# jedison-github/gentun

Hardware: AMD Instinct MI355X
Metric: candidates/hour + best val-acc@genN, Genetic-CNN CIFAR-10 1/2/4/8 GPU (higher is better)
Workload: dtype fp32

## Files before the change

### csrc/hip/cnn_args.h

```cpp
#pragma once
#include "common.h"

template <typename F>
static void lds_limit(F* fn, size_t bytes) {
  if (bytes > 65536) (void)hipFuncSetAttribute(reinterpret_cast<const void*>(fn), hipFuncAttributeMaxDynamicSharedMemorySize,
                                         (int)bytes);
}

struct GroupRec {
  int g;
  int in_mask;
  int out_mask;
  int pad;
};

#define GT_MAXSLOT 8

struct ConvArgs {
  const void* in[GT_MAXSLOT];
  const void* mask;
  const int64_t* gather;
  const StepState* st;
  void* out[GT_MAXSLOT];
  const void* out_mask[GT_MAXSLOT];
  const uint16_t* w;
  const float* bias;
  const GroupRec* gtab;
  int n_in, n_out, acc_flags, relu;
  int G, B, H, W, Cinp, Coutp, KH, KW, TH;
  int ngroups;
  void* xsum;
  int dbg;
  int epi_bf16;
  int prec;
  long wps;
  int cbb;
  void* pool_y;
  uint8_t* pool_mask;
  void* unpool_x1;
  const int* unpool_sel;
  int cout_real;
  int Hr, Wr;
  int wino;
  int wfrag;
};

__device__ __forceinline__ GroupRec group_rec(const GroupRec* gtab, int y, int n_in, int n_out, int acc,
                                              const void* const* out_mask) {
  if (gtab) return gtab[y];
  GroupRec r;
  r.g = y;
  r.in_mask = (1 << n_in) - 1;
  int rm = 0;
  for (int k = 0; k < n_out; ++k)
    if (out_mask && out_mask[k]) rm |= 1 << k;
  r.out_mask = ((1 << n_out) - 1) | ((acc & 0xff) << 8) | (rm << 16);
  r.pad = 0;
  return r;
}

struct WgradArgs {
  const void* in[GT_MAXSLOT];
  const int64_t* gather;
  const StepState* st;
  const void* dz;
  float* part_w;
  float* part_b;
  const GroupRec* gtab;
  int n_in;
  int G, B, H, W, Cinp, Coutp, KH, KW, S, pps;
  int ngroups;
  int prec;
  int cout_real;
};

__device__ __forceinline__ bool pos_bits(uint32_t h) { return h != 0u && h < 0x8000u; }
```

### csrc/hip/cnn_conv_fast.hip

```cpp
#include "conv_fast_host.h"

FastSwitches g_fast;

static int swap_switch(int& sw, int v) {
  const int old = sw;
  sw = v;
  return old;
}

extern "C" int gt_conv_set_s2in_ct1(int on) { return swap_switch(g_fast.s2in_ct1, on); }

extern "C" int gt_conv_set_regepi(int on) { return swap_switch(g_fast.regepi, on); }

extern "C" int gt_conv_set_smallq(int on) { return swap_switch(g_fast.smallq, on); }

static int smallq_th(const ConvArgs* a, int TH, int THMIN) {
  if (!g_fast.smallq) return TH;
  int th = TH;
  while (th > THMIN && (long)a->ngroups * a->B * (a->H / th) < g_fast.smallq_wg) th >>= 1;
  return th;
}

static bool pk_ok(const ConvArgs* a, int nt) {
  const int last = a->cout_real - 16 * (nt - 1);
  return a->prec == 1 && a->cout_real > 0 && last >= 1 && last <= 4;
}

static const std::vector<ConvRow>& conv_rows() {
  static const std::vector<ConvRow> rows = {
    {8, 4, {tile<5, 5, 1, 32, 4, 2, 3, 2, 1, 1>(IF_TH | IF_PK), tile<5, 5, 1, 32, 4, 2, 3, 2, 1>(IF_TH),
            tile<5, 5, 1, 32, 8, 2, 3, 4, 1, 1>(IF_PK), tile<5, 5, 1, 32, 8, 2, 3, 4, 1>()}},
    {8, 4, {tile<3, 3, 3, 32, 4, 2, 3, 2, 1, 1>(IF_TH | IF_PK), tile<3, 3, 3, 32, 4, 2, 3, 2, 1>(IF_TH),
            tile<3, 3, 3, 32, 8, 2, 3, 4, 1, 1>(IF_PK), tile<3, 3, 3, 32, 8, 2, 3, 4, 1>()}},
    {8, 2, {tile<5, 5, 3, 16, 4, 4, 7, 4, 1>(IF_TH), ct1<5, 5, 3, 16, 2, 4, 7, 4>(IF_TH), ct1<5, 5, 3, 16, 8, 4, 7, 4, 0>()}},
    {8, 2, {tile<3, 3, 7, 16, 4, 4, 7, 4, 1>(IF_TH), ct1<3, 3, 7, 16, 2, 4, 7, 4>(IF_TH), ct1<3, 3, 7, 16, 8, 4, 7, 4, 0>()}},
    {8, 4, {ct1<5, 5, 7, 16, 4, 2, 3, 4>(IF_S2CT1 | IF_TH), ct1<5, 5, 7, 16, 8, 2, 3, 4>(IF_S2CT1),
            tile<5, 5, 7, 16, 8, 2, 3, 4, 1, 1>(IF_PK), tile<5, 5, 7, 16, 8, 2, 3, 4, 1>()}},
    {8, 8, {tile<5, 5, 7, 8, 8, 7, 13, 7, 1>()}},
    {8, 8, {tile<3, 3, 13, 8, 8, 7, 13, 7, 1>()}},
    {8, 8, {tile<5, 5, 13, 8, 8, 4, 7, 4, 1>()}},
    {8, 8, {tile<5, 5, 1, 32, 8, 4, 8, 4, 1>()}},
    {4, 4, {ct1<3, 3, 8, 32, 4, 4, 8, 4, 0>()}},
    {8, 8, {ct1<5, 5, 8, 16, 8, 8, 16, 8, 0>()}},
    {8, 8, {ct1<3, 3, 16, 16, 8, 8, 16, 8, 0>()}},
    {4, 4, {tile<5, 5, 16, 16, 4, 4, 8, 4, 1>()}},
    {8, 8, {tile<5, 5, 16, 8, 8, 16, 32, 8, 1>()}},
    {8, 8, {tile<3, 3, 32, 8, 8, 16, 32, 8, 1>()}},
    {4, 4, {tile<5, 5, 32, 8, 4, 8, 16, 4, 1>()}},
    {8, 8, {tile<5, 5, 1, 32, 8, 2, 3, 4, 0>()}},
    {8, 8, {tile<3, 3, 3, 32, 8, 2, 3, 4, 0>()}},
    {16, 16, {tile<5, 5, 3, 16, 16, 4, 7, 4, 0>()}},
    {16, 16, {tile<3, 3, 7, 16, 16, 4, 7, 8, 0>()}},
    {16, 16, {tile<5, 5, 7, 16, 16, 2, 3, 4, 0>()}},
    {8, 8, {tile<5, 5, 7, 8, 8, 7, 13, 7, 0>()}},
    {8, 8, {tile<3, 3, 13, 8, 8, 7, 13, 7, 0>()}},
    {8, 8, {tile<5, 5, 13, 8, 8, 4, 7, 4, 0>()}},
  };
  return rows;
}

struct ConvChoice {
  const ConvKernel* k;
  dim3 grid;
  unsigned block;
  size_t lds;
};

static bool variant_ok(const ConvArgs* a, const ConvRow& r, const ConvVariant& v) {
  return (!(v.cond & IF_TH) || smallq_th(a, r.hmod, r.thmin) == v.k.TH) && (!(v.cond & IF_PK) || pk_ok(a, v.k.NT)) &&
         (!(v.cond & IF_RE) || g_fast.regepi) && (!(v.cond & IF_S2CT1) || g_fast.s2in_ct1);
}

static bool select_conv(const ConvArgs* a, ConvChoice* c) {
  if (a->mask) return false;
  for (const std::vector<ConvRow>* rows : {&conv_rows(), &conv_rows_ext()})
    for (const ConvRow& r : *rows) {
      const ConvKernel& g = r.v[0].k;
      if (a->KH != g.KH || a->KW != g.KW || a->Cinp != g.NCBI * 8 || a->W != g.W || a->Coutp != g.NCO * 8 ||
          a->prec != g.PREC || a->H % r.hmod != 0)
        continue;
      for (const ConvVariant& v : r.v)
        if (variant_ok(a, r, v)) {
          *c = {&v.k, dim3(a->B * (a->H / v.k.TH), a->ngroups), (unsigned)v.k.NWV * 64,
                (size_t)(a->epi_bf16 != 0 ? v.k.lds_fwd : v.k.lds_bwd)};
          return true;
        }
    }
  return false;
}

static int launch_fast(const void* fn, dim3 grid, unsigned block, size_t lds, const void* args, hipStream_t stream) {
  lds_limit(fn, lds);
  void* kargs[] = {const_cast<void*>(args)};
  (void)hipLaunchKernel(fn, grid, dim3(block), kargs, lds, stream);
  return (int)hipGetLastError();
}

extern "C" int gt_conv_wino(const ConvArgs* a, hipStream_t stream, int probe);

extern "C" int gt_conv_fast(const ConvArgs* a, hipStream_t stream) {
  if (a->wino) return gt_conv_wino(a, stream, 0);
  if (a->mask) return -100;
  if (a->prec != 0 && a->prec != 1) return -1;
  ConvChoice c;
  if (!select_conv(a, &c)) return -100;
  return launch_fast(c.k->fn, c.grid, c.block, c.lds, a, stream);
}

static int probe_rows(const ConvArgs* a) {
  if (a->wino) {
    const int rc = gt_conv_wino(a, nullptr, 1);
    return rc >= 1000 ? rc - 1000 : 0;
  }
  ConvChoice c;
  return select_conv(a, &c) ? c.k->TH : 0;
}

extern "C" int gt_conv_fast_probe(const ConvArgs* a) {
  const int th = probe_rows(a);
  return th % 2 == 0 ? th : 0;
}

extern "C" int gt_conv_fast_probe_any(const ConvArgs* a) { return probe_rows(a) > 0 ? 1 : 0; }

struct ConvSel {
  int KH, KW, NCBI, W, TH, NT, NCO, NWV, PREC, PK, RE, CTX, SCH, lds_fwd, lds_bwd;
  int gx, gy, gz, block, lds;
};
extern "C" int gt_conv_fast_select(const ConvArgs* a, ConvSel* s) {
  ConvChoice c;
  if (a->wino || (a->prec != 0 && a->prec != 1) || !select_conv(a, &c)) return 0;
  const ConvKernel& k = *c.k;
  *s = {k.KH, k.KW, k.NCBI, k.W, k.TH, k.NT, k.NCO, k.NWV, k.PREC, k.PK, k.RE, k.CTX, k.SCH, k.lds_fwd, k.lds_bwd,
        (int)c.grid.x, (int)c.grid.y, (int)c.grid.z, (int)c.block, (int)c.lds};
  return 1;
}
extern "C" size_t gt_sizeof_conv_sel() { return sizeof(ConvSel); }

__global__ void __launch_bounds__(256) wgrad_reduce_kernel(WgradArgs a) {
  const GroupRec gr = group_rec(a.gtab, blockIdx.y, a.n_in, 0, 0, nullptr);
  const int g = gr.g;
  const long kd = (long)a.KH * a.KW * a.Cinp;
  const long n = (long)a.Coutp * kd;
  const long gs = (long)a.G * n;
  float* pw = a.part_w + (long)g * n;
  const long i4 = ((long)blockIdx.x * 256 + threadIdx.x) * 4;
  if (i4 < n) {
    float4 acc = make_float4(0.f, 0.f, 0.f, 0.f);
    int sp = 0;
    for (; sp + 8 <= a.S; sp += 8) {
      float4 v[8];
#pragma unroll
      for (int k = 0; k < 8; ++k) v[k] = *reinterpret_cast<const float4*>(pw + (long)(sp + k) * gs + i4);
#pragma unroll
      for (int k = 0; k < 8; ++k) { acc.x += v[k].x; acc.y += v[k].y; acc.z += v[k].z; acc.w += v[k].w; }
    }
    for (; sp < a.S; ++sp) {
      const float4 v = *reinterpret_cast<const float4*>(pw + (long)sp * gs + i4);
      acc.x += v.x; acc.y += v.y; acc.z += v.z; acc.w += v.w;
    }
    *reinterpret_cast<float4*>(pw + i4) = acc;
  }
  if (blockIdx.x == 0 && a.part_b) {
    float* pb = a.part_b + (long)g * a.Coutp;
    for (int i = threadIdx.x; i < a.Coutp; i += 256) {
      float acc = 0.f;
      for (int sp = 0; sp < a.S; ++sp) acc += pb[(long)sp * a.G * a.Coutp + i];
      pb[i] = acc;
    }
  }
}

extern "C" int gt_wgrad_reduce(const WgradArgs* a, hipStream_t stream) {
  const long n = (long)a->Coutp * a->KH * a->KW * a->Cinp;
  if (n % 4 || a->S < 2) return -1;
  dim3 grid((unsigned)((n / 4 + 255) / 256), a->ngroups);
  hipLaunchKernelGGL(wgrad_reduce_kernel, grid, dim3(256), 0, stream, *a);
  return (int)hipGetLastError();
}

extern "C" int gt_wgrad_set_nb(int nb) { return swap_switch(g_fast.wgrad_nb, nb); }

extern "C" int gt_wgrad_set_nz(int nz) { return swap_switch(g_fast.wgrad_nz, nz); }

static int wgrad_nz(const WgradArgs* a) {
  const int force = g_fast.wgrad_nz;
  if (force == 1 || force == 2 || force == 4 || force == 8) return force;
  const int blocks = a->S * a->ngroups;
  return blocks < 64 ? 4 : blocks < 160 ? 2 : 1;
}

static bool wgrad_pk_ok(const WgradArgs* a, int mt) {
  const int last = a->cout_real - 16 * (mt - 1);
  return a->cout_real > 0 && last >= 1 && last <= 4;
}

static const std::vector<WgradRow>& wgrad_rows() {
  static const std::vector<WgradRow> rows = {
    wgrad_f32<5, 5, 1, 3, 32, 8, 4, 1>(),
    wgrad_f32<3, 3, 3, 3, 32, 4, 4, 1>(),
    wgrad_f32<5, 5, 3, 7, 16, 4, 8, 1>(),
    wgrad_f32<3, 3, 7, 7, 16, 4, 8, 1>(),
    wgrad_f32z<5, 5, 7, 13, 8, 4, 8, 4>(),
    wgrad_f32z<3, 3, 13, 13, 8, 4, 8, 4>(),
    wgrad_f32<5, 5, 1, 8, 32, 4, 4, 1>(),
    wgrad_f32<3, 3, 8, 8, 32, 2, 8, 1>(),
    wgrad_f32z<5, 5, 8, 16, 16, 2, 8, 7>(),
    wgrad_f32z<3, 3, 16, 16, 16, 2, 8, 4>(),
    wgrad_f32z<5, 5, 16, 32, 8, 4, 8, 13>(),
    wgrad_f32z<3, 3, 32, 32, 8, 4, 8, 10>(),
    wgrad_bf16<5, 5, 1, 3, 32, 8, 4, 1>(),
    wgrad_bf16<3, 3, 3, 3, 32, 8, 4, 1>(),
    wgrad_bf16<5, 5, 3, 7, 16, 16, 8, 2>(),
    wgrad_bf16<3, 3, 7, 7, 16, 16, 8, 2>(),
  };
  return rows;
}

static const WgradRow* wgrad_row(int KH, int KW, int Cinp, int Coutp, int H, int W, int prec) {
  for (const std::vector<WgradRow>* rows : {&wgrad_rows(), &wgrad_rows_ext()})
    for (const WgradRow& r : *rows)
      if (KH == r.KH && KW == r.KW && Cinp == r.NCBI * 8 && Coutp == r.NCBO * 8 && W == r.W && prec == r.PREC &&
          H % r.R == 0)
        return &r;
  return nullptr;
}

struct WgradChoice {
  const WgradKernel* k;
  dim3 grid;
  unsigned block;
};

static bool select_wgrad(const WgradArgs* a, WgradChoice* c) {
  const WgradRow* r = wgrad_row(a->KH, a->KW, a->Cinp, a->Coutp, a->H, a->W, a->prec);
  if (!r || a->pps % (r->R * r->W) != 0) return false;
  const int nz = r->NZ ? r->NZ : wgrad_nz(a);
  const int pk = r->PREC == 1 && wgrad_pk_ok(a, (r->NCBO * 8 + 15) / 16) ? 1 : 0;
  int nw = r->NW, nb = 1;
  if (r->NZ == 0 && nz == 2) nb = r->NB;
  else if (r->NZ == 0 && nz == 8) nw = 4;
  else if (nz == 1) nb = (g_fast.wgrad_nb ? g_fast.wgrad_nb : r->NB) == 1 ? 1 : 2;
  for (const WgradKernel& k : r->k)
    if (k.NW == nw && k.NB == nb && k.PK == pk && k.NZ == nz) {
      *c = {&k, dim3(a->S, a->ngroups, nz), (unsigned)nw * 64};
      return true;
    }
  return false;
}

extern "C" int gt_wgrad_fast_band(int KH, int KW, int Cinp, int Coutp, int H, int W, int prec) {
  const WgradRow* r = wgrad_row(KH, KW, Cinp, Coutp, H, W, prec);
  return r ? r->R * r->W : 0;
}

extern "C" int gt_wgrad_fast_splits(int KH, int KW, int Cinp, int Coutp, int H, int W, int prec) {
  (void)KH; (void)KW; (void)Cinp; (void)Coutp; (void)H;
  if (prec == 1) {
    return W >= 32 ? 32 : W <= 8 ? 4 : 8;
  }
  return W >= 32 ? 16 : 3;
}

extern "C" int gt_wgrad_fast(const WgradArgs* a, hipStream_t stream) {
  if (a->prec != 0 && a->prec != 1) return -1;
  WgradChoice c;
  if (!select_wgrad(a, &c)) return -100;
  return launch_fast(c.k->fn, c.grid, c.block, 0, a, stream);
}

struct WgradSel {
  int KH, KW, NCBI, NCBO, W, R, NW, NB, PK, NZ, PREC;
  int gx, gy, gz, block, lds;
};
extern "C" int gt_wgrad_fast_select(const WgradArgs* a, WgradSel* s) {
  WgradChoice c;
  if (!select_wgrad(a, &c)) return 0;
  const WgradKernel& k = *c.k;
  *s = {k.KH, k.KW, k.NCBI, k.NCBO, k.W, k.R, k.NW, k.NB, k.PK, k.NZ, k.PREC,
        (int)c.grid.x, (int)c.grid.y, (int)c.grid.z, (int)c.block, 0};
  return 1;
}
extern "C" size_t gt_sizeof_wgrad_sel() { return sizeof(WgradSel); }

extern "C" int gt_conv_frag_order(int KH, int KW, int NCBI, int W, int prec, int* out, int n) {
  const int NCH = KH * KW * NCBI;
  const bool parts = prec == 1 && NCBI == 7 && W == 16 && KH == 3 && KW == 3;
  for (int e = 0; e < n; ++e) {
    int kk, cb;
    if (e >= NCH) { out[e] = -1; continue; }
    if (parts) {
      const int E0 = KH * KW * 4;
      if (e < E0) { kk = e >> 2; cb = e & 3; }
      else { const int e1 = e - E0; kk = e1 / 3; cb = 4 + e1 - kk * 3; }
    } else {
      kk = e / NCBI; cb = e - kk * NCBI;
    }
    out[e] = kk * NCBI + cb;
  }
  return (NCH + 3) / 4;
}

struct FragSeg {
  const float* w;
  uint16_t* dst;
  const int* order;
  long ps;
  int Q, Cop, Cip, KH, KW;
  int NT, NKS, NCBIc;
  int dgrad;
  int npl;
};

struct FragArgs {
  const FragSeg* segs;
  const int2* blocks;
};

__global__ void __launch_bounds__(256) conv_wfrag_kernel(FragArgs a) {
  const int2 blk = a.blocks[blockIdx.x];
  const FragSeg s = a.segs[blk.x];
  const long item = (long)blk.y + threadIdx.x;
  if (item >= (long)s.Q * s.NT * s.NKS * 64) return;
  const int lane = (int)(item & 63);
  long r = item >> 6;
  const int ks = (int)(r % s.NKS); r /= s.NKS;
  const int t = (int)(r % s.NT);
  const int q = (int)(r / s.NT);
  const int row = t * 16 + (lane & 15), e = ks * 4 + (lane >> 4);
  const int nat = s.order[e];
  float v[8];
#pragma unroll
  for (int j = 0; j < 8; ++j) v[j] = 0.f;
  if (nat >= 0) {
    const int kk = nat / s.NCBIc, cb = nat - kk * s.NCBIc;
    const int kh = kk / s.KW, kw = kk - kh * s.KW;
    if (!s.dgrad && row < s.Cop) {
      const float* src = s.w + ((((long)q * s.Cop + row) * s.KH + kh) * s.KW + kw) * s.Cip + cb * 8;
#pragma unroll
      for (int j = 0; j < 8; ++j) v[j] = src[j];
    } else if (s.dgrad && row < s.Cip) {
      const int khl = s.KH - 1 - kh, kwl = s.KW - 1 - kw;
#pragma unroll
      for (int j = 0; j < 8; ++j)
        v[j] = s.w[((((long)q * s.Cop + cb * 8 + j) * s.KH + khl) * s.KW + kwl) * s.Cip + row];
    }
  }
  uint16_t* d = s.dst + item * 8;
  if (s.npl == 1) {
    *reinterpret_cast<uint4*>(d) = pack8(v);
    return;
  }
  uint4 p0, p1, p2;
  split8(v, p0, p1, p2);
  *reinterpret_cast<uint4*>(d) = p0;
  *reinterpret_cast<uint4*>(d + s.ps) = p1;
  *reinterpret_cast<uint4*>(d + 2 * s.ps) = p2;
}

extern "C" int gt_conv_wfrag(const void* av, int nblocks, hipStream_t stream) {
  if (nblocks < 1) return 0;
  hipLaunchKernelGGL(conv_wfrag_kernel, dim3(nblocks), dim3(256), 0, stream, *static_cast<const FragArgs*>(av));
  return (int)hipGetLastError();
}

extern "C" size_t gt_sizeof_frag_seg() { return sizeof(FragSeg); }
```

### csrc/hip/conv_fast_host.h

```cpp
#pragma once
#include <initializer_list>
#include <vector>

#include "conv_fast_impl.h"

struct FastSwitches {
  int s2in_ct1 = 1;
  int regepi = 1;
  int smallq = 1;
  long smallq_wg = 300;
  int wgrad_nb = 0;
  int wgrad_nz = 0;
};
extern FastSwitches g_fast;

struct ConvKernel {
  int KH, KW, NCBI, W, TH, NT, NCO, NWV, PREC, PK, RE, CTX, SCH;
  int lds_fwd, lds_bwd;
  const void* fn;
};

template <int KH, int KW, int NCBI, int W, int TH, int NT, int NCO, int NWV, int PREC, int PK = 0, int RE = 0,
          int CTX = 0, int SCH = 0>
static ConvKernel conv_kernel() {
  static_assert((NCO * 8 + 15) / 16 == NT, "NT co tiles of 16 cover the NCO chunks of 8 channels");
  using Cfg = FastCfg<KH, KW, NCBI, W, TH, NT, NCO, PREC>;
  return {KH, KW, NCBI, W, TH, NT, NCO, NWV, PREC, PK, RE, CTX, SCH, (int)Cfg::lds(true), (int)Cfg::lds(false),
          reinterpret_cast<const void*>(&conv_fast_kernel<KH, KW, NCBI, W, TH, NT, NCO, NWV, PREC, PK, RE, CTX, SCH>)};
}

enum : int {
  IF_TH = 1,
  IF_PK = 2,
  IF_RE = 4,
  IF_S2CT1 = 8,
};

struct ConvVariant {
  int cond;
  ConvKernel k;
};
typedef std::vector<ConvVariant> ConvVariants;

template <int KH, int KW, int NCBI, int W, int TH, int NT, int NCO, int NWV, int PREC, int PK = 0>
static ConvVariants tile(int cond = 0) {
  ConvVariants v;
  if (PREC == 1 && W % 16 == 0) v.push_back({cond | IF_RE, conv_kernel<KH, KW, NCBI, W, TH, NT, NCO, NWV, PREC, PK, 1>()});
  v.push_back({cond, conv_kernel<KH, KW, NCBI, W, TH, NT, NCO, NWV, PREC, PK, 0>()});
  return v;
}

template <int KH, int KW, int NCBI, int W, int TH, int NT, int NCO, int NWV, int SCH = 1>
static ConvVariants ct1(int cond = 0) {
  return {{cond, conv_kernel<KH, KW, NCBI, W, TH, NT, NCO, NWV, 1, 0, 1, 1, SCH>()}};
}

struct ConvRow {
  int hmod, thmin;
  ConvVariants v;
  ConvRow(int hmod_, int thmin_, std::initializer_list<ConvVariants> parts) : hmod(hmod_), thmin(thmin_) {
    for (const ConvVariants& p : parts) v.insert(v.end(), p.begin(), p.end());
  }
};

struct WgradKernel {
  int KH, KW, NCBI, NCBO, W, R, NW, NB, PK, NZ, PREC;
  const void* fn;
};

template <int KH, int KW, int NCBI, int NCBO, int W, int R, int NW, int NB, int PK = 0, int NZ = 1>
static WgradKernel wgrad_kernel_f32() {
  return {KH, KW, NCBI, NCBO, W, R, NW, NB, PK, NZ, 1,
          reinterpret_cast<const void*>(&wgrad_fast_f32_kernel<KH, KW, NCBI, NCBO, W, R, NW, NB, PK, NZ>)};
}
template <int KH, int KW, int NCBI, int NCBO, int W, int R, int NW, int NB>
static WgradKernel wgrad_kernel_bf16() {
  return {KH, KW, NCBI, NCBO, W, R, NW, NB, 0, 1, 0,
          reinterpret_cast<const void*>(&wgrad_fast_kernel<KH, KW, NCBI, NCBO, W, R, NW, NB>)};
}

struct WgradRow {
  int KH, KW, NCBI, NCBO, W, R, NW, PREC;
  int NB;
  int NZ;
  std::vector<WgradKernel> k;
};

template <int KH, int KW, int NCBI, int NCBO, int W, int R, int NW, int NB>
static WgradRow wgrad_f32() {
  return {KH, KW, NCBI, NCBO, W, R, NW, 1, NB, 0,
          {wgrad_kernel_f32<KH, KW, NCBI, NCBO, W, R, NW, 1, 0>(), wgrad_kernel_f32<KH, KW, NCBI, NCBO, W, R, NW, 1, 1>(),
           wgrad_kernel_f32<KH, KW, NCBI, NCBO, W, R, NW, 2, 0>(), wgrad_kernel_f32<KH, KW, NCBI, NCBO, W, R, NW, 2, 1>(),
           wgrad_kernel_f32<KH, KW, NCBI, NCBO, W, R, NW, NB, 0, 2>(), wgrad_kernel_f32<KH, KW, NCBI, NCBO, W, R, NW, NB, 1, 2>(),
           wgrad_kernel_f32<KH, KW, NCBI, NCBO, W, R, NW, 1, 0, 4>(), wgrad_kernel_f32<KH, KW, NCBI, NCBO, W, R, NW, 1, 1, 4>(),
           wgrad_kernel_f32<KH, KW, NCBI, NCBO, W, R, 4, 1, 0, 8>(), wgrad_kernel_f32<KH, KW, NCBI, NCBO, W, R, 4, 1, 1, 8>()}};
}
template <int KH, int KW, int NCBI, int NCBO, int W, int R, int NW, int NZ>
static WgradRow wgrad_f32z() {
  return {KH, KW, NCBI, NCBO, W, R, NW, 1, 1, NZ,
          {wgrad_kernel_f32<KH, KW, NCBI, NCBO, W, R, NW, 1, 0, NZ>(), wgrad_kernel_f32<KH, KW, NCBI, NCBO, W, R, NW, 1, 1, NZ>()}};
}
template <int KH, int KW, int NCBI, int NCBO, int W, int R, int NW, int NB>
static WgradRow wgrad_bf16() {
  return {KH, KW, NCBI, NCBO, W, R, NW, 0, NB, 1,
          {wgrad_kernel_bf16<KH, KW, NCBI, NCBO, W, R, NW, 1>(), wgrad_kernel_bf16<KH, KW, NCBI, NCBO, W, R, NW, 2>()}};
}

const std::vector<ConvRow>& conv_rows_ext();
const std::vector<WgradRow>& wgrad_rows_ext();
```

### csrc/hip/conv_fast_impl.h

```cpp
#pragma once

#include <algorithm>
#include <cstdio>
#include <cstdlib>
#include <type_traits>

#include "cnn_args.h"


__device__ __forceinline__ int opaque_i(int x) {
  asm volatile("" : "+v"(x));
  return x;
}

template <int KH, int KW, int NCBI, int W, int PREC>
struct S2Parts {
  static constexpr bool on = PREC == 1 && NCBI == 7 && W == 16 && KH == 3 && KW == 3;
  static constexpr int e0 = KH * KW * 4;
};

template <int KH, int KW, int NCBI, int W, int TH, int NT, int NCO, int PREC>
struct FastCfg {
  static constexpr int NPL = PREC ? GT_NPL_F32 : 1;
  static constexpr int PW = W + KW - 1;
  static constexpr int NP = (TH + KH - 1) * PW * NCBI;
  static constexpr int NCBP = NCBI + ((NCBI & 1) ? 0 : 1);
  static constexpr int NPIX = (TH + KH - 1) * PW;
  static constexpr int PPR = (S2Parts<KH, KW, NCBI, W, PREC>::on || NCBI == 3) ? 5 : (NCBI % 2 == 0) ? (NCBI == 4 ? 4 : 2) : 6;
  static constexpr int PP2 = 2 * NPIX + ((PPR - (2 * NPIX) % 8) + 8) % 8;
  static constexpr int TP = TH * W;
  static constexpr int OROW = NT * 16 + 4;
  static constexpr int OROWB = NT * 16 + 8;
  static constexpr int NPL_ = PREC ? GT_NPL_F32 : 1;
  static constexpr long OTILE = (long)TP * OROW * 4;
  static constexpr long LDS_PM = (long)NPIX * NCBP * 16 * NPL_ > OTILE ? (long)NPIX * NCBP * 16 * NPL_ : OTILE;
  static constexpr long LDS_PR = (long)((NCBI + 1) / 2) * PP2 * 16 * NPL_ > OTILE ? (long)((NCBI + 1) / 2) * PP2 * 16 * NPL_ : OTILE;
  static constexpr long LDS_CU = 160 * 1024;
  static constexpr bool PAIR = PREC == 1 && NCBI >= 2 && LDS_CU / LDS_PR >= LDS_CU / LDS_PM;
  static constexpr int PXS = PAIR ? 2 : NCBP;
  static constexpr int NPP = PAIR ? ((NCBI + 1) / 2) * PP2 : NPIX * NCBP;
  __host__ __device__ static constexpr int cbo(int cb) { return PAIR ? (cb >> 1) * PP2 + (cb & 1) : cb; }
  static size_t lds(bool fwd) {
    const size_t p = (size_t)NPP * 16 * NPL;
    const size_t o = (fwd && !PREC) ? (size_t)TP * OROWB * 2 : (size_t)TP * OROW * 4;
    return p > o ? p : o;
  }
};

template <int TH, int W, int NCO, int NTH, int PREC, typename LD>
__device__ __forceinline__ void fused_pool(const ConvArgs& a, LD ld, int g, int b, int h0, int tid) {
  typedef typename ActT<PREC>::T AT;
  constexpr int WO = W / 2, NPP = (TH / 2) * WO * NCO;
  static_assert(TH % 2 == 0 && W % 2 == 0, "pooled tiles need even rows / columns");
  const int Ho = a.H >> 1;
  const long n = (long)g * a.B + b;
  for (int i = tid; i < NPP; i += NTH) {
    const int cb = i % NCO, pp = i / NCO, pr = pp / WO, pc = pp - pr * WO;
    const int p0 = 2 * pr * W + 2 * pc;
    float m[8], t[8];
    int arg[8] = {0, 0, 0, 0, 0, 0, 0, 0};
    ld(p0, cb, m);
    const int offs[3] = {1, W, W + 1};
#pragma unroll
    for (int q = 0; q < 3; ++q) {
      ld(p0 + offs[q], cb, t);
#pragma unroll
      for (int j = 0; j < 8; ++j)
        if (t[j] > m[j]) { m[j] = t[j]; arg[j] = q + 1; }
    }
    const long o = ((n * Ho + (h0 >> 1) + pr) * WO + pc) * (NCO * 8) + cb * 8;
    st_chunk(static_cast<AT*>(a.pool_y) + o, m);
    if (a.pool_mask) {
      uint32_t lo = 0, hi = 0;
#pragma unroll
      for (int j = 0; j < 4; ++j) lo |= (uint32_t)(arg[j] | (m[j] > 0.f ? 4 : 0)) << (8 * j);
#pragma unroll
      for (int j = 0; j < 4; ++j) hi |= (uint32_t)(arg[4 + j] | (m[4 + j] > 0.f ? 4 : 0)) << (8 * j);
      *reinterpret_cast<uint2*>(a.pool_mask + o) = make_uint2(lo, hi);
    }
  }
}

template <typename AT>
__device__ __forceinline__ void unpool_chunk(const ConvArgs& a, int g, long n, int h, int w, int cb, const float* v) {
  const int Cp = a.Coutp, H2 = 2 * a.H, W2 = 2 * a.W;
  const long o = ((n * a.H + h) * a.W + w) * Cp + cb * 8;
  const uint2 mk = *reinterpret_cast<const uint2*>(a.pool_mask + o);
  AT* dst = static_cast<AT*>((a.unpool_sel && a.unpool_sel[g]) ? a.unpool_x1 : a.pool_y);
#pragma unroll
  for (int me = 0; me < 4; ++me) {
    float out[8];
#pragma unroll
    for (int j = 0; j < 8; ++j) {
      const uint32_t b = ((j < 4 ? mk.x : mk.y) >> (8 * (j & 3))) & 0xffu;
      out[j] = ((int)(b & 3u) == me && (b & 4u)) ? v[j] : 0.f;
    }
    st_chunk(dst + ((n * H2 + 2 * h + (me >> 1)) * W2 + 2 * w + (me & 1)) * Cp + cb * 8, out);
  }
}

template <int CT, int PG, int PK, int W, int NCO, bool POOLABLE>
__device__ __forceinline__ void f32_epi_regs(const ConvArgs& a, const GroupRec& gr, int b, int h0,
                                             const f32x4_t (&acc)[CT][PG], int wco, int pgw, int lane);

template <int KH, int KW, int NCBI, int W, int TH, int NT, int NCO, int NWV = 4, int PREC = 0, int PK = 0, int RE = 0,
          int CTX = 0, int SCH = 0>
__global__ void __launch_bounds__(NWV * 64)
__attribute__((amdgpu_waves_per_eu(PREC ? 2 : (NWV == 8 ? 4 : (NT >= 4 ? (NCBI >= 7 ? 2 : 3) : 4)))))
conv_fast_kernel(ConvArgs a) {
  typedef typename ActT<PREC>::T AT;
  constexpr int NPL = PREC ? GT_NPL_F32 : 1;
  constexpr int NTH = NWV * 64;
  constexpr int PH = TH + KH - 1, PW = W + KW - 1;
  constexpr int NP = PH * PW * NCBI;
  using FCL = FastCfg<KH, KW, NCBI, W, TH, NT, NCO, PREC>;
  constexpr int NCBP = FCL::NCBP;
  constexpr int PXS = FCL::PXS;
  constexpr int NPP = FCL::NPP;
  auto pslot = [&](int i) {
    if constexpr (NCBP == NCBI && !FCL::PAIR) return i;
    else return (i / NCBI) * PXS + FCL::cbo(i % NCBI);
  };
  constexpr int NPT = (NP + NTH - 1) / NTH;
  constexpr int NCH = KH * KW * NCBI;
  constexpr int NKS = (NCH + 3) / 4;
  constexpr bool PARTS = S2Parts<KH, KW, NCBI, W, PREC>::on;
  auto ent = [&](int e, int& kk, int& cb) {
    if constexpr (PARTS) {
      constexpr int E0 = S2Parts<KH, KW, NCBI, W, PREC>::e0;
      if (e < E0) { kk = e >> 2; cb = e & 3; }
      else { const int e1 = e - E0; kk = e1 / 3; cb = 4 + e1 - kk * 3; }
    } else {
      kk = e / NCBI; cb = e - kk * NCBI;
    }
  };
  constexpr int TP = TH * W;
  constexpr int NPG = TP / 16;
  constexpr int CT = CTX ? CTX : PK ? NT : ((NT >= 2 && NT % 2 == 0) ? 2 : 1);
  constexpr int WC = NT / CT;
  constexpr int WP = NWV / WC;
  constexpr int PG = NPG / WP;
  constexpr int PFM = PREC ? ((CTX == 1 && !SCH && NWV == 4 && NCBI <= 7) ? 3 : 2) : 4;
  constexpr int PF = NKS < PFM ? NKS : PFM;
  constexpr bool SCHED = SCH && PREC != 0 && NKS <= 64;
  constexpr int RA = SCHED ? PF + 1 : PF;
  static_assert(NPG % WP == 0 && NT % CT == 0 && WC * WP == NWV, "tile shape");
  static_assert(!PK || (PREC == 1 && WC == 1), "packed last tile: fp32, every wave owns all co tiles");
  static_assert(W % 16 == 0 || 16 % W == 0, "pixel groups must tile image rows");

  using FC = FastCfg<KH, KW, NCBI, W, TH, NT, NCO, PREC>;
  constexpr int OROW = FC::OROW, OROWB = FC::OROWB;
  extern __shared__ __attribute__((aligned(16))) uint4 smem[];
  uint4* patch = smem;
  __shared__ int coff[NKS * 4];

  const int tid = threadIdx.x, wave = tid >> 6, lane = tid & 63, kq = lane >> 4, l16 = lane & 15;
  const int nbx = gridDim.x;
  const int total = nbx * gridDim.y;
  int lin = blockIdx.y * nbx + blockIdx.x;
  if ((total & 7) == 0) lin = (lin & 7) * (total >> 3) + (lin >> 3);
  const int by = lin / nbx, bx = lin - by * nbx;
  const int nband = (a.H + TH - 1) / TH;
  const int b = bx / nband;
  const int h0 = (bx - b * nband) * TH;
  const GroupRec gr = group_rec(a.gtab, by, a.n_in, a.n_out, a.acc_flags, a.out_mask);
  const int g = gr.g;
  const long img = (long)a.H * W * NCBI * 8;

  const int wco = (wave % WC) * CT;
  const int pgw = (wave / WC) * PG;
  const uint16_t* wrow[CT];
  bool wok[CT];
#pragma unroll
  for (int t = 0; t < CT; ++t) {
    if (PK && t == CT - 1) {
      const int co = (wco + t) * 16 + (l16 >> 2), pl = l16 & 3;
      wok[t] = pl < 3 && co < a.cout_real;
      wrow[t] = a.wfrag ? a.w + (((long)g * NT + wco + t) * NKS * 64 + kq * 16 + (l16 >> 2)) * 8 + (wok[t] ? pl : 0) * a.wps
                        : a.w + ((long)g * (NCO * 8) + (wok[t] ? co : 0)) * (NCH * 8) + (wok[t] ? pl : 0) * a.wps;
      continue;
    }
    const int co = (wco + t) * 16 + l16;
    wok[t] = co < NCO * 8;
    wrow[t] = a.wfrag ? a.w + (((long)g * NT + wco + t) * NKS * 64 + lane) * 8
                      : a.w + ((long)g * (NCO * 8) + (wok[t] ? co : 0)) * (NCH * 8);
  }
  uint4 areg[RA][CT][NPL];
  auto load_a = [&](int s, uint4 (*dst)[NPL]) {
    const int e = ((a.dbg & 8) ? 0 : s * 4) + kq;
    int c = e;
    if constexpr (PARTS) {
      int kk, cb;
      ent(e, kk, cb);
      c = kk * NCBI + cb;
    }
    const bool fr = a.wfrag != 0;
#pragma unroll
    for (int t = 0; t < CT; ++t) {
      const bool ok = fr ? (!(PK && t == CT - 1) || wok[t]) : (wok[t] && e < NCH);
      const long off = fr ? (long)((a.dbg & 8) ? 0 : s) * 512 : (long)c * 8;
#pragma unroll
      for (int p = 0; p < ((PK && t == CT - 1) ? 1 : NPL); ++p)
        dst[t][p] = *reinterpret_cast<const uint4*>(ok ? (const void*)(wrow[t] + p * a.wps + off) : (const void*)gt_zero8);
    }
  };
  auto mma = [&](int t, const uint4* af, const uint4* bf, f32x4_t c) {
    if (PK && t == CT - 1) {
      c = mfma16(af[0], bf[2], c);
      c = mfma16(af[0], bf[1], c);
      return mfma16(af[0], bf[0], c);
    }
    return mfma_np<NPL>(af, bf, c);
  };

  const long gimg = ((long)g * a.B + b) * img;
  const int n_src = a.gather ? 1 : __builtin_popcount(gr.in_mask);
  const AT* src0 = a.gather ? static_cast<const AT*>(a.in[0]) + a.gather[((long)a.st->cur_step * a.G + g) * a.B + b] * img
                            : static_cast<const AT*>(a.in[__builtin_ctz(gr.in_mask | 0x100) & 7]) + gimg;
  long poff[NPT];
  bool pok[NPT];
#pragma unroll
  for (int j = 0; j < NPT; ++j) {
    const int i = tid + NTH * j;
    const int cb = i % NCBI, pix = i / NCBI;
    const int pr = pix / PW, pc = pix % PW;
    const int hh = h0 - KH / 2 + pr, ww = pc - KW / 2;
    pok[j] = i < NP && hh >= 0 && hh < a.H && ww >= 0 && ww < W;
    poff[j] = ((long)hh * W + ww) * (NCBI * 8) + cb * 8;
  }
  if (a.dbg & 4) {
#pragma unroll
    for (int j = 0; j < NPT; ++j)
#pragma unroll
      for (int p = 0; p < NPL; ++p)
        if (tid + NTH * j < NP) patch[p * NPP + pslot(tid + NTH * j)] = make_uint4(0, 0, 0, 0);
  } else if (!PREC && n_src == 1) {
    uint4 v[NPT];
#pragma unroll
    for (int j = 0; j < NPT; ++j)
      v[j] = *reinterpret_cast<const uint4*>(pok[j] ? (const void*)(src0 + poff[j]) : (const void*)gt_zero8);
#pragma unroll
    for (int j = 0; j < NPT; ++j)
      if (tid + NTH * j < NP) patch[pslot(tid + NTH * j)] = v[j];
  } else {
    constexpr int JB = NPT < 5 ? NPT : 5;
#pragma unroll
    for (int j0 = 0; j0 < NPT; j0 += JB) {
      float acc8[JB][8];
#pragma unroll
      for (int j = 0; j < JB; ++j)
#pragma unroll
        for (int e = 0; e < 8; ++e) acc8[j][e] = 0.f;
      if (n_src == 1) {
#pragma unroll
        for (int j = 0; j < JB; ++j)
          if (j0 + j < NPT && pok[j0 + j]) ld_chunk(src0 + poff[j0 + j], acc8[j]);
      } else {
        int m = gr.in_mask & 0xff;
        while (m) {
          const int k0 = __builtin_ctz(m);
          m &= m - 1;
          const bool two = m != 0;
          const int k1 = two ? __builtin_ctz(m) : k0;
          if (two) m &= m - 1;
          const AT* s0 = static_cast<const AT*>(a.in[k0]) + gimg;
          const AT* s1 = static_cast<const AT*>(a.in[k1]) + gimg;
          float t0[JB][8], t1[JB][8];
#pragma unroll
          for (int j = 0; j < JB; ++j) {
#pragma unroll
            for (int e = 0; e < 8; ++e) t0[j][e] = t1[j][e] = 0.f;
            if (j0 + j < NPT && pok[j0 + j]) {
              ld_chunk(s0 + poff[j0 + j], t0[j]);
              if (two) ld_chunk(s1 + poff[j0 + j], t1[j]);
            }
          }
#pragma unroll
          for (int j = 0; j < JB; ++j)
#pragma unroll
            for (int e = 0; e < 8; ++e) acc8[j][e] += t0[j][e];
          if (two) {
#pragma unroll
            for (int j = 0; j < JB; ++j)
#pragma unroll
              for (int e = 0; e < 8; ++e) acc8[j][e] += t1[j][e];
          }
        }
      }
#pragma unroll
      for (int j = 0; j < JB; ++j) {
        const int i = tid + NTH * (j0 + j);
        if (j0 + j >= NPT || i >= NP) continue;
        if (PREC) {
          uint4 p0, p1, p2;
          split8(acc8[j], p0, p1, p2);
          patch[pslot(i)] = p0;
          patch[NPP + pslot(i)] = p1;
          patch[2 * NPP + pslot(i)] = p2;
        } else {
          patch[pslot(i)] = pack8(acc8[j]);
        }
      }
    }
  }
  if (a.xsum && n_src > 1) {
    __syncthreads();
    AT* xo = static_cast<AT*>(a.xsum) + ((long)g * a.B + b) * img + (long)h0 * W * NCBI * 8;
    for (int i = tid; i < TH * W * NCBI; i += NTH) {
      const int cb = i % NCBI, pix = i / NCBI;
      const int r = pix / W, c = pix % W;
      if (h0 + r >= a.H) continue;
      const int pi = ((r + KH / 2) * PW + c + KW / 2) * PXS + FCL::cbo(cb);
      if (PREC) {
        float f[8];
        join8(patch[pi], patch[NPP + pi], patch[2 * NPP + pi], f);
        st_chunk(xo + (long)i * 8, f);
      } else {
        *reinterpret_cast<uint4*>(xo + (long)i * 8) = patch[pi];
      }
    }
  }
  for (int c = tid; c < NKS * 4; c += NTH) {
    int kk, cb;
    ent(c, kk, cb);
    coff[c] = c < NCH ? ((kk / KW) * PW + (kk % KW)) * PXS + FCL::cbo(cb) : 0;
  }
#pragma unroll
  for (int s = 0; s < PF; ++s) load_a(s, areg[s]);
  float bias_v[CT][4];
#pragma unroll
  for (int t = 0; t < CT; ++t)
#pragma unroll
    for (int i = 0; i < 4; ++i) {
      const int co = (PK && t == CT - 1) ? (i == 0 ? (wco + t) * 16 + kq : NCO * 8) : (wco + t) * 16 + kq * 4 + i;
      bias_v[t][i] = (a.bias && co < NCO * 8) ? a.bias[(long)g * (NCO * 8) + co] : 0.f;
    }
  __syncthreads();

  const int lbase = ((l16 / W) * PW + (l16 % W)) * PXS;
  int gbase;
  {
    const int p = pgw * 16;
    gbase = ((p / W) * PW + (p % W)) * PXS;
  }
  f32x4_t acc[CT][PG];
#pragma unroll
  for (int t = 0; t < CT; ++t)
#pragma unroll
    for (int h = 0; h < PG; ++h) acc[t][h] = (f32x4_t){0.f, 0.f, 0.f, 0.f};

  auto koff = [&](int s) {
    const int c = s * 4 + kq;
    int kk, cb;
    ent(c, kk, cb);
    return c < NCH ? ((kk / KW) * PW + (kk % KW)) * PXS + FCL::cbo(cb) : 0;
  };
  auto load_b = [&](int s, uint4 (*dst)[NPL]) {
    const uint4* pb = patch + lbase + gbase + (SCHED ? koff(s) : coff[s * 4 + kq]);
#pragma unroll
    for (int h = 0; h < PG; ++h) {
      const int p = h * 16;
#pragma unroll
      for (int q = 0; q < NPL; ++q) dst[h][q] = pb[q * NPP + ((p / W) * PW + (p % W)) * PXS];
    }
  };
  if (!(a.dbg & 1)) {
    if constexpr (PREC != 0 && NKS > 64) {
      static_assert(PF == 2, "k-step pairs need a 2-deep weight prefetch");
      uint4 bfr[2][PG][NPL];
      load_b(0, bfr[0]);
      auto kstep = [&](int s, auto par) {
        constexpr int P = decltype(par)::value;
        load_b(min(s + 1, NKS - 1), bfr[P ^ 1]);
#pragma unroll
        for (int t = 0; t < CT; ++t)
#pragma unroll
          for (int h = 0; h < PG; ++h) acc[t][h] = mma(t, areg[P][t], bfr[P][h], acc[t][h]);
        load_a(min(s + PF, NKS - 1), areg[P]);
      };
      for (int s = 0; s < NKS; s += 2) {
        kstep(s, std::integral_constant<int, 0>());
        if (s + 1 < NKS) kstep(s + 1, std::integral_constant<int, 1>());
      }
    } else if constexpr (SCHED) {
      uint4 bfr[2][PG][NPL];
      load_b(0, bfr[0]);
#pragma unroll
      for (int s = 0; s < NKS; ++s) {
        if (s + 1 < NKS) load_b(s + 1, bfr[(s + 1) & 1]);
        __builtin_amdgcn_sched_barrier(0);
#pragma unroll
        for (int t = 0; t < CT; ++t)
#pragma unroll
          for (int h = 0; h < PG; ++h) acc[t][h] = mma(t, areg[s % RA][t], bfr[s & 1][h], acc[t][h]);
        __builtin_amdgcn_sched_barrier(0);
        if (s + PF < NKS) load_a(s + PF, areg[(s + PF) % RA]);
        __builtin_amdgcn_sched_barrier(0);
      }
    } else if constexpr (PREC != 0) {
      uint4 bfr[2][PG][NPL];
      load_b(0, bfr[0]);
#pragma unroll
      for (int s = 0; s < NKS; ++s) {
        if (s + 1 < NKS) load_b(s + 1, bfr[(s + 1) & 1]);
#pragma unroll
        for (int t = 0; t < CT; ++t)
#pragma unroll
          for (int h = 0; h < PG; ++h) acc[t][h] = mma(t, areg[s % PF][t], bfr[s & 1][h], acc[t][h]);
        if (s + PF < NKS) load_a(s + PF, areg[s % PF]);
      }
    } else {
#pragma unroll
      for (int s = 0; s < NKS; ++s) {
        uint4 bfr[PG][NPL];
        load_b(s, bfr);
#pragma unroll
        for (int t = 0; t < CT; ++t)
#pragma unroll
          for (int h = 0; h < PG; ++h) acc[t][h] = mma(t, areg[s % PF][t], bfr[h], acc[t][h]);
        if (s + PF < NKS) load_a(s + PF, areg[s % PF]);
      }
    }
  }

  if constexpr (RE != 0 && PREC != 0 && W % 16 == 0) {
    constexpr bool PL = TH % 2 == 0 && PG % (2 * (W / 16)) == 0;
    f32_epi_regs<CT, PG, PK, W, NCO, PL>(a, gr, b, h0, acc, wco, pgw, lane);
    return;
  }
  if (a.epi_bf16 && !PREC) {
    __syncthreads();
    uint16_t* ot = reinterpret_cast<uint16_t*>(smem);
#pragma unroll
    for (int t = 0; t < CT; ++t) {
      const int co0 = (wco + t) * 16 + kq * 4;
#pragma unroll
      for (int h = 0; h < PG; ++h) {
        const int p = (pgw + h) * 16 + l16;
        const bool pad0 = a.Hr > 0 && (h0 + p / W >= a.Hr || p % W >= a.Wr);
        float v[4];
#pragma unroll
        for (int i = 0; i < 4; ++i) {
          v[i] = acc[t][h][i] + bias_v[t][i];
          if (a.relu) v[i] = fmaxf(v[i], 0.f);
          if (pad0) v[i] = 0.f;
        }
        *reinterpret_cast<uint2*>(ot + p * OROWB + co0) = pack4(v);
      }
    }
    __syncthreads();
    const long obase = (((long)g * a.B + b) * a.H + h0) * W * (NCO * 8);
    if (!(a.dbg & 2))
#pragma unroll
    for (int j = 0; j < (TP * NCO + NTH - 1) / NTH; ++j) {
      const int i = tid + NTH * j;
      if (i >= TP * NCO) break;
      const int p = i / NCO, cb = i - p * NCO;
      const uint4 val = *reinterpret_cast<const uint4*>(ot + p * OROWB + cb * 8);
#pragma unroll
      for (int k = 0; k < GT_MAXSLOT; ++k)
        if ((gr.out_mask >> k) & 1) *reinterpret_cast<uint4*>(static_cast<uint16_t*>(a.out[k]) + obase + (long)i * 8) = val;
    }
    if constexpr (TH % 2 == 0)
      if (a.pool_y && ((gr.out_mask >> 24) & 1))
        fused_pool<TH, W, NCO, NTH, 0>(
            a, [&](int p, int cb, float* f) { unpack8(*reinterpret_cast<const uint4*>(ot + p * OROWB + cb * 8), f); },
            g, b, h0, tid);
    return;
  }
  __syncthreads();
  float* otile = reinterpret_cast<float*>(smem);
#pragma unroll
  for (int t = 0; t < CT; ++t) {
    const int co0 = (wco + t) * 16 + kq * 4;
#pragma unroll
    for (int h = 0; h < PG; ++h) {
      const int p = (pgw + h) * 16 + l16;
      const bool pad0 = a.Hr > 0 && (h0 + p / W >= a.Hr || p % W >= a.Wr);
      if (PK && t == CT - 1) {
        float s0 = acc[t][h][0] + acc[t][h][1] + acc[t][h][2] + bias_v[t][0];
        if (a.relu) s0 = fmaxf(s0, 0.f);
        if (pad0) s0 = 0.f;
        float* orow = otile + p * OROW + (wco + t) * 16;
        orow[kq] = s0;
        orow[4 + kq] = 0.f;
        orow[8 + kq] = 0.f;
        orow[12 + kq] = 0.f;
        continue;
      }
      float4 v;
      v.x = acc[t][h][0] + bias_v[t][0];
      v.y = acc[t][h][1] + bias_v[t][1];
      v.z = acc[t][h][2] + bias_v[t][2];
      v.w = acc[t][h][3] + bias_v[t][3];
      if (a.relu) { v.x = fmaxf(v.x, 0.f); v.y = fmaxf(v.y, 0.f); v.z = fmaxf(v.z, 0.f); v.w = fmaxf(v.w, 0.f); }
      if (pad0) v = make_float4(0.f, 0.f, 0.f, 0.f);
      *reinterpret_cast<float4*>(otile + p * OROW + co0) = v;
    }
  }
  __syncthreads();
  if (a.dbg & 2) return;
  const long obase = (((long)g * a.B + b) * a.H + h0) * W * (NCO * 8);
#pragma unroll
  for (int j = 0; j < (TP * NCO + NTH - 1) / NTH; ++j) {
    const int i = tid + NTH * j;
    if (i >= TP * NCO) break;
    const int p = i / NCO, cb = i - p * NCO;
    const float4 lo = *reinterpret_cast<const float4*>(otile + p * OROW + cb * 8);
    const float4 hi = *reinterpret_cast<const float4*>(otile + p * OROW + cb * 8 + 4);
    const float v[8] = {lo.x, lo.y, lo.z, lo.w, hi.x, hi.y, hi.z, hi.w};
    const long off = obase + (long)i * 8;
    if ((gr.out_mask >> 25) & 1) {
      unpool_chunk<AT>(a, g, (long)g * a.B + b, h0 + p / W, p % W, cb, v);
      continue;
    }
    for (int k = 0; k < GT_MAXSLOT; ++k) {
      if (!((gr.out_mask >> k) & 1)) continue;
      AT* dst = static_cast<AT*>(a.out[k]) + off;
      float sum[8];
#pragma unroll
      for (int e = 0; e < 8; ++e) sum[e] = v[e];
      if ((gr.out_mask >> (8 + k)) & 1) {
        float o[8];
        ld_chunk(dst, o);
#pragma unroll
        for (int e = 0; e < 8; ++e) sum[e] += o[e];
      }
      if ((gr.out_mask >> (16 + k)) & 1) {
        float m[8];
        ld_chunk(static_cast<const AT*>(a.out_mask[k]) + off, m);
#pragma unroll
        for (int e = 0; e < 8; ++e) sum[e] = m[e] > 0.f ? sum[e] : 0.f;
      }
      st_chunk(dst, sum);
    }
  }
  if constexpr (TH % 2 == 0)
    if (a.pool_y && ((gr.out_mask >> 24) & 1))
      fused_pool<TH, W, NCO, NTH, PREC>(
          a, [&](int p, int cb, float* f) { load8f(otile + p * OROW + cb * 8, f); }, g, b, h0, tid);
}

template <int CT, int PG, int PK, int W, int NCO, bool POOLABLE>
__device__ __forceinline__ void f32_epi_regs(const ConvArgs& a, const GroupRec& gr, int b, int h0,
                                             const f32x4_t (&acc)[CT][PG], int wco, int pgw, int lane) {
  constexpr int COP = NCO * 8, RG = W / 16;
  const int kq = lane >> 4, l16 = lane & 15;
  const long oimg = (long)a.H * W * COP;

  if (a.dbg & 2) return;
  const int g = gr.g;
  const long n = (long)g * a.B + b;
  const long obase = n * oimg + (long)h0 * W * COP;
  const bool pool = a.pool_y && ((gr.out_mask >> 24) & 1);
  const bool unpool = (gr.out_mask >> 25) & 1;
  float val[CT][PG][4];
  bool cok[CT];
#pragma unroll
  for (int t = 0; t < CT; ++t) {
    const bool pkt = PK && t == CT - 1;
    const int co0 = (wco + t) * 16 + kq * 4;
    cok[t] = co0 < COP;
    float bv[4] = {0.f, 0.f, 0.f, 0.f};
    if (a.bias) {
      if (pkt) {
        const int co = (wco + t) * 16 + kq;
        bv[0] = co < COP ? a.bias[(long)g * COP + co] : 0.f;
      } else if (co0 < COP) {
        const float4 q = *reinterpret_cast<const float4*>(a.bias + (long)g * COP + co0);
        bv[0] = q.x; bv[1] = q.y; bv[2] = q.z; bv[3] = q.w;
      }
    }
#pragma unroll
    for (int h = 0; h < PG; ++h) {
      if (pkt) {
        float s0 = acc[t][h][0] + acc[t][h][1] + acc[t][h][2] + bv[0];
        if (a.relu) s0 = fmaxf(s0, 0.f);
#pragma unroll
        for (int i = 0; i < 4; ++i) {
          const float o = __shfl(s0, l16 + 16 * i, 64);
          val[t][h][i] = kq == 0 ? o : 0.f;
        }
      } else {
#pragma unroll
        for (int i = 0; i < 4; ++i) {
          float v = acc[t][h][i] + bv[i];
          if (a.relu) v = fmaxf(v, 0.f);
          val[t][h][i] = v;
        }
      }
    }
  }
  if (a.Hr > 0 && !unpool) {
#pragma unroll
    for (int h = 0; h < PG; ++h) {
      const int p = (pgw + h) * 16 + l16;
      if (h0 + p / W >= a.Hr || p % W >= a.Wr) {
#pragma unroll
        for (int t = 0; t < CT; ++t)
#pragma unroll
          for (int i = 0; i < 4; ++i) val[t][h][i] = 0.f;
      }
    }
  }
  auto off_of = [&](int t, int h) {
    return obase + (long)((pgw + h) * 16 + l16) * COP + (wco + t) * 16 + kq * 4;
  };
  if (unpool) {
    uint32_t mk[CT][PG];
#pragma unroll
    for (int t = 0; t < CT; ++t)
#pragma unroll
      for (int h = 0; h < PG; ++h)
        mk[t][h] = *reinterpret_cast<const uint32_t*>(a.pool_mask + (cok[t] ? off_of(t, h) : 0));
    float* dst = static_cast<float*>((a.unpool_sel && a.unpool_sel[g]) ? a.unpool_x1 : a.pool_y);
    const int H2 = 2 * a.H, W2 = 2 * W;
#pragma unroll
    for (int t = 0; t < CT; ++t) {
      if (!cok[t]) continue;
#pragma unroll
      for (int h = 0; h < PG; ++h) {
        const int p = (pgw + h) * 16 + l16;
        const int hh = h0 + p / W, ww = p % W;
#pragma unroll
        for (int me = 0; me < 4; ++me) {
          float o[4];
#pragma unroll
          for (int i = 0; i < 4; ++i) {
            const uint32_t bb = (mk[t][h] >> (8 * i)) & 0xffu;
            o[i] = ((int)(bb & 3u) == me && (bb & 4u)) ? val[t][h][i] : 0.f;
          }
          *reinterpret_cast<float4*>(dst + ((n * H2 + 2 * hh + (me >> 1)) * W2 + 2 * ww + (me & 1)) * COP +
                                     (wco + t) * 16 + kq * 4) = make_float4(o[0], o[1], o[2], o[3]);
        }
      }
    }
  } else {
    for (int k = 0; k < GT_MAXSLOT; ++k) {
      if (!((gr.out_mask >> k) & 1)) continue;
      float* dst = static_cast<float*>(a.out[k]);
      float o[CT][PG][4];
#pragma unroll
      for (int t = 0; t < CT; ++t)
#pragma unroll
        for (int h = 0; h < PG; ++h)
#pragma unroll
          for (int i = 0; i < 4; ++i) o[t][h][i] = val[t][h][i];
      if ((gr.out_mask >> (8 + k)) & 1) {
        float4 q[CT][PG];
#pragma unroll
        for (int t = 0; t < CT; ++t)
#pragma unroll
          for (int h = 0; h < PG; ++h) q[t][h] = *reinterpret_cast<const float4*>(dst + (cok[t] ? off_of(t, h) : 0));
#pragma unroll
        for (int t = 0; t < CT; ++t)
#pragma unroll
          for (int h = 0; h < PG; ++h) {
            o[t][h][0] += q[t][h].x; o[t][h][1] += q[t][h].y; o[t][h][2] += q[t][h].z; o[t][h][3] += q[t][h].w;
          }
      }
      if ((gr.out_mask >> (16 + k)) & 1) {
        const float* mp = static_cast<const float*>(a.out_mask[k]);
        float4 q[CT][PG];
#pragma unroll
        for (int t = 0; t < CT; ++t)
#pragma unroll
          for (int h = 0; h < PG; ++h) q[t][h] = *reinterpret_cast<const float4*>(mp + (cok[t] ? off_of(t, h) : 0));
#pragma unroll
        for (int t = 0; t < CT; ++t)
#pragma unroll
          for (int h = 0; h < PG; ++h) {
            o[t][h][0] = q[t][h].x > 0.f ? o[t][h][0] : 0.f; o[t][h][1] = q[t][h].y > 0.f ? o[t][h][1] : 0.f;
            o[t][h][2] = q[t][h].z > 0.f ? o[t][h][2] : 0.f; o[t][h][3] = q[t][h].w > 0.f ? o[t][h][3] : 0.f;
          }
      }
#pragma unroll
      for (int t = 0; t < CT; ++t) {
        if (!cok[t]) continue;
#pragma unroll
        for (int h = 0; h < PG; ++h)
          *reinterpret_cast<float4*>(dst + off_of(t, h)) = make_float4(o[t][h][0], o[t][h][1], o[t][h][2], o[t][h][3]);
      }
    }
  }
  if constexpr (POOLABLE) {
    if (pool) {
      const int Ho = a.H >> 1, Wo = W >> 1;
#pragma unroll
      for (int t = 0; t < CT; ++t) {
#pragma unroll
        for (int h = 0; h < PG; ++h) {
          if ((h / RG) % 2) continue;
          float m[4];
          uint32_t mk = 0;
#pragma unroll
          for (int i = 0; i < 4; ++i) {
            const float v00 = val[t][h][i], v10 = val[t][h + RG][i];
            const float v01 = __shfl(v00, lane + 1, 64), v11 = __shfl(v10, lane + 1, 64);
            float mm = v00;
            int arg = 0;
            if (v01 > mm) { mm = v01; arg = 1; }
            if (v10 > mm) { mm = v10; arg = 2; }
            if (v11 > mm) { mm = v11; arg = 3; }
            m[i] = mm;
            mk |= (uint32_t)(arg | (mm > 0.f ? 4 : 0)) << (8 * i);
          }
          if ((l16 & 1) || !cok[t]) continue;
          const int p = (pgw + h) * 16 + l16;
          const int pr = (h0 + p / W) >> 1, pc = (p % W) >> 1;
          const long o = ((n * Ho + pr) * Wo + pc) * COP + (wco + t) * 16 + kq * 4;
          *reinterpret_cast<float4*>(static_cast<float*>(a.pool_y) + o) = make_float4(m[0], m[1], m[2], m[3]);
          if (a.pool_mask) *reinterpret_cast<uint32_t*>(a.pool_mask + o) = mk;
        }
      }
    }
  }
}



typedef __attribute__((ext_vector_type(4))) short wf_short4_t;
typedef __attribute__((ext_vector_type(8))) short wf_short8_t;

__device__ __forceinline__ uint4 tr_pair(const char* lo_addr, const char* hi_addr) {
  typedef __attribute__((address_space(3))) wf_short4_t lds_s4;
  const wf_short4_t lo = __builtin_amdgcn_ds_read_tr16_b64_v4i16((lds_s4*)(lo_addr));
  const wf_short4_t hi = __builtin_amdgcn_ds_read_tr16_b64_v4i16((lds_s4*)(hi_addr));
  const wf_short8_t v = __builtin_shufflevector(lo, hi, 0, 1, 2, 3, 4, 5, 6, 7);
  return __builtin_bit_cast(uint4, v);
}

__device__ __attribute__((aligned(16))) uint4 wf_zero16[1];

typedef __attribute__((address_space(3))) void wf_lvoid_t;

__device__ __forceinline__ void wf_glds16(const void* src, const void* lds_wave_base) {
  const uint32_t l = __builtin_amdgcn_readfirstlane((uint32_t)(uintptr_t)(wf_lvoid_t*)lds_wave_base);
  uint32_t keep;
  asm volatile("s_mov_b32 %0, m0\n\ts_mov_b32 m0, %2\n\ts_nop 0\n\tglobal_load_lds_dwordx4 %1, off\n\ts_mov_b32 m0, %0"
               : "=&s"(keep) : "v"(src), "s"(l) : "memory");
}

template <int KH, int KW, int NCBI, int NCBO, int W, int R, int NW, int NB>
__global__ void __launch_bounds__(NW * 64) wgrad_fast_kernel(WgradArgs a) {
  constexpr int NT_ = NW * 64;
  constexpr int PW = W + KW - 1, PR = R + KH - 1;
  constexpr int NCH = KH * KW * NCBI;
  constexpr int NKT = (NCH + 1 + 1) / 2;
  constexpr int MT = (NCBO * 8 + 15) / 16;
  constexpr int TPW = (NKT + NW - 1) / NW;
  constexpr int KS = R * W / 32;
  constexpr int XCH = PR * PW * NCBI;
  constexpr int DCH = R * W * NCBO;
  constexpr int XT = (XCH + NT_ - 1) / NT_, DT = (DCH + NT_ - 1) / NT_;
  constexpr int XCR = (XCH + 63) / 64 * 64, DCR = (DCH + 63) / 64 * 64;
  constexpr int XROW = NCBI * 16, DROW = NCBO * 16;
  static_assert(R * W % 32 == 0 && (W == 16 || W == 32), "bands must be whole 32-pixel K-steps");

  __shared__ __attribute__((aligned(16))) uint4 xs[NB][XCR];
  __shared__ __attribute__((aligned(16))) uint4 ds[NB][DCR];

  const int tid = threadIdx.x, wave = tid >> 6, lane = tid & 63;
  const int s = blockIdx.x;
  const GroupRec gr = group_rec(a.gtab, blockIdx.y, a.n_in, 0, 0, nullptr);
  const int g = gr.g;
  const int nbi = a.H / R;
  const int bps = a.pps / (R * W);
  const int band0 = s * bps;
  const int band1 = min(band0 + bps, a.B * nbi);
  const long img_in = (long)a.H * W * NCBI * 8, img_out = (long)a.H * W * NCBO * 8;
  const int first_in = __builtin_ctz(gr.in_mask | 0x100);
  const bool single = __builtin_popcount(gr.in_mask) == 1 || a.gather;
  const long fold_off = (long)g * a.B * img_in;

  auto issue = [&](int band, int buf) {
    const int b = band / nbi, h0 = (band - b * nbi) * R;
    const uint16_t* src0 = a.gather ? static_cast<const uint16_t*>(a.in[0]) +
                                          a.gather[((long)a.st->cur_step * a.G + g) * a.B + b] * img_in
                                    : static_cast<const uint16_t*>(a.in[first_in & 7]) + fold_off + (long)b * img_in;
#pragma unroll
    for (int j = 0; j < XT; ++j) {
      const int i = tid + NT_ * j;
      const int cb = i % NCBI, pix = i / NCBI;
      const int hh = h0 - KH / 2 + pix / PW, ww = pix % PW - KW / 2;
      const bool ok = i < XCH && hh >= 0 && hh < a.H && ww >= 0 && ww < W;
      const long off = ((long)hh * W + ww) * (NCBI * 8) + cb * 8;
      if (single) {
        if (NT_ * j + 64 * wave < XCR)
          wf_glds16(ok ? (const void*)(src0 + off) : (const void*)wf_zero16, &xs[buf][NT_ * j + 64 * wave]);
      } else if (i < XCH) {
        float sum[8] = {0, 0, 0, 0, 0, 0, 0, 0}, t8[8];
        if (ok) {
#pragma unroll
          for (int k = 0; k < GT_MAXSLOT; ++k) {
            if (!((gr.in_mask >> k) & 1)) continue;
            unpack8(*reinterpret_cast<const uint4*>(static_cast<const uint16_t*>(a.in[k]) + fold_off +
                                                    (long)b * img_in + off), t8);
#pragma unroll
            for (int e = 0; e < 8; ++e) sum[e] += t8[e];
          }
        }
        xs[buf][i] = pack8(sum);
      }
    }
    const char* dsrc = reinterpret_cast<const char*>(static_cast<const uint16_t*>(a.dz) + (long)g * a.B * img_out +
                                                     (long)b * img_out + (long)h0 * W * NCBO * 8);
#pragma unroll
    for (int j = 0; j < DT; ++j) {
      const int i = tid + NT_ * j;
      if (NT_ * j + 64 * wave < DCR)
        wf_glds16(i < DCH ? (const void*)(dsrc + (long)i * 16) : (const void*)wf_zero16, &ds[buf][NT_ * j + 64 * wave]);
    }
  };

  const int gq = lane >> 4, q = (lane >> 2) & 3, p = lane & 3, l16 = lane & 15;
  const int px0 = 8 * gq + q;
  const int prow = px0 / W, pcol = px0 % W;
  const int xlane = (prow * PW + pcol) * XROW;
  const int dlane = px0 * DROW + p * 8;
  int xoff[TPW];
#pragma unroll
  for (int t = 0; t < TPW; ++t) {
    const int n = wave + NW * t;
    int c = 2 * n + (p >> 1);
    if (c >= NCH) c = 0;
    const int kk = c / NCBI, cb = c % NCBI;
    xoff[t] = xlane + ((kk / KW) * PW + (kk % KW)) * XROW + cb * 16 + (p & 1) * 8;
  }
  const bool ones_lane = l16 == (NCH & 1) * 8;

  f32x4_t acc[MT][TPW];
#pragma unroll
  for (int m = 0; m < MT; ++m)
#pragma unroll
    for (int t = 0; t < TPW; ++t) acc[m][t] = (f32x4_t){0.f, 0.f, 0.f, 0.f};

  if (band0 < band1) issue(band0, 0);
  int cur = 0;
  for (int band = band0; band < band1; ++band, cur ^= (NB - 1)) {
    asm volatile("s_waitcnt vmcnt(0)" ::: "memory");
    __syncthreads();
    if (NB == 2 && band + 1 < band1) issue(band + 1, cur ^ 1);
    const char* xb = reinterpret_cast<const char*>(xs[cur]);
    const char* db = reinterpret_cast<const char*>(ds[cur]) + dlane;
#pragma unroll
    for (int ks = 0; ks < KS; ++ks) {
      const int xrow_off = ((ks * 32) / W) * PW * XROW;
      uint4 afr[MT];
#pragma unroll
      for (int m = 0; m < MT; ++m) {
        const char* d0 = db + ks * 32 * DROW + m * 32;
        afr[m] = tr_pair(d0, d0 + 4 * DROW);
      }
#pragma unroll
      for (int t = 0; t < TPW; ++t) {
        const int n = wave + NW * t;
        if (n >= NKT) continue;
        const char* x0 = xb + xrow_off + xoff[t];
        uint4 bfr = tr_pair(x0, x0 + 4 * XROW);
        if (n == NCH / 2 && ones_lane) bfr = make_uint4(0x3f803f80u, 0x3f803f80u, 0x3f803f80u, 0x3f803f80u);
#pragma unroll
        for (int m = 0; m < MT; ++m) acc[m][t] = mfma16(afr[m], bfr, acc[m][t]);
      }
    }
    if (NB == 1 && band + 1 < band1) {
      __syncthreads();
      issue(band + 1, 0);
    }
  }

  const int kq = lane >> 4;
  constexpr int Kdim = NCH * 8;
#pragma unroll
  for (int t = 0; t < TPW; ++t) {
    const int n = wave + NW * t;
    if (n >= NKT) continue;
    const int col = n * 16 + l16;
#pragma unroll
    for (int m = 0; m < MT; ++m)
#pragma unroll
      for (int i = 0; i < 4; ++i) {
        const int co = m * 16 + kq * 4 + i;
        if (co >= a.Coutp) continue;
        if (col < Kdim)
          a.part_w[(((long)s * a.G + g) * a.Coutp + co) * Kdim + col] = acc[m][t][i];
        else if (col == Kdim && a.part_b)
          a.part_b[((long)s * a.G + g) * a.Coutp + co] = acc[m][t][i];
      }
  }
}

template <int KH, int KW, int NCBI, int NCBO, int W, int R, int NW, int NB, int PK = 0, int NZ = 1>
__global__ void __launch_bounds__(NW * 64) wgrad_fast_f32_kernel(WgradArgs a) {
  constexpr int NPL = GT_NPL_F32;
  constexpr int NT_ = NW * 64;
  constexpr int PW = W + KW - 1, PR = R + KH - 1;
  constexpr int NCH = KH * KW * NCBI;
  constexpr int NKT = (NCH + 1 + 1) / 2;
  constexpr int MT = (NCBO * 8 + 15) / 16;
  constexpr int TPW = ((NKT + NZ - 1) / NZ + NW - 1) / NW;
  constexpr int KS = R * W / 32;
  constexpr int XCH = PR * PW * NCBI;
  constexpr int DCH = R * W * NCBO;
  constexpr int XT = (XCH + NT_ - 1) / NT_, DT = (DCH + NT_ - 1) / NT_;
  constexpr int NCBIP0 = NCBI + ((NCBI & 1) ? 0 : 1), NCBOP0 = NCBO + ((NCBO & 1) ? 0 : 1);
  constexpr bool PADOK = (long)NB * NPL * (PR * PW * NCBIP0 + R * W * NCBOP0) * 16 + (long)NB * R * W * 32 <= 160 * 1024;
  constexpr int NCBIP = PADOK ? NCBIP0 : NCBI, NCBOP = PADOK ? NCBOP0 : NCBO;
  constexpr int XCHL = PR * PW * NCBIP, DCHL = R * W * NCBOP;
  constexpr int XROW = NCBIP * 16, DROW = NCBOP * 16;
  auto xslot = [&](int i) {
    if constexpr (NCBIP == NCBI) return i;
    else return (i / NCBI) * NCBIP + i % NCBI;
  };
  auto dslot = [&](int i) {
    if constexpr (NCBOP == NCBO) return i;
    else return (i / NCBO) * NCBOP + i % NCBO;
  };
  constexpr bool MOUT = NZ > 1;
  static_assert(R * W % 32 == 0 && (W == 8 || W == 16 || W == 32), "bands must be whole 32-pixel K-steps");

  __shared__ __attribute__((aligned(16))) uint4 xs[NB][NPL][XCHL];
  __shared__ __attribute__((aligned(16))) uint4 ds[NB][NPL][DCHL];
  constexpr int PKC = 2 * (MT - 1);
  constexpr int PKR = PK ? R * W : 1;
  __shared__ __attribute__((aligned(16))) uint4 dpk[NB][PKR][2];
  static_assert(!PK || PKC < NCBO, "packed tile inside the staged dz chunks");

  const int tid = threadIdx.x, wave = tid >> 6, lane = tid & 63;
  const int s = blockIdx.x;
  const int nz0 = NZ > 1 ? (int)blockIdx.z * NW * TPW : 0;
  const GroupRec gr = group_rec(a.gtab, blockIdx.y, a.n_in, 0, 0, nullptr);
  const int g = gr.g;
  const int nbi = a.H / R;
  const int bps = a.pps / (R * W);
  const int band0 = s * bps;
  const int band1 = min(band0 + bps, a.B * nbi);
  const long img_in = (long)a.H * W * NCBI * 8, img_out = (long)a.H * W * NCBO * 8;
  const long fold_off = (long)g * a.B * img_in;
  const int n_src = a.gather ? 1 : __builtin_popcount(gr.in_mask);
  const float* in0 = static_cast<const float*>(a.in[__builtin_ctz(gr.in_mask | 0x100) & 7]);

  float xr[XT][8], dr[DT][8];
  auto load = [&](int band) {
    const int b = band / nbi, h0 = (band - b * nbi) * R;
    const long boff = fold_off + (long)b * img_in;
    const float* src0 = a.gather ? static_cast<const float*>(a.in[0]) +
                                       a.gather[((long)a.st->cur_step * a.G + g) * a.B + b] * img_in
                                 : in0 + boff;
#pragma unroll
    for (int j = 0; j < XT; ++j) {
      const int i = tid + NT_ * j;
      const int cb = i % NCBI, pix = i / NCBI;
      const int hh = h0 - KH / 2 + pix / PW, ww = pix % PW - KW / 2;
      const bool ok = i < XCH && hh >= 0 && hh < a.H && ww >= 0 && ww < W;
      const long off = ((long)hh * W + ww) * (NCBI * 8) + cb * 8;
      if (n_src == 1) {
#pragma unroll
        for (int e = 0; e < 8; ++e) xr[j][e] = 0.f;
        if (ok) load8f(src0 + off, xr[j]);
      } else {
#pragma unroll
        for (int e = 0; e < 8; ++e) xr[j][e] = 0.f;
        for (int k = 0; k < GT_MAXSLOT; ++k) {
          if (!((gr.in_mask >> k) & 1)) continue;
          float t8[8];
          load8f_or0(static_cast<const float*>(a.in[k]) + boff + off, ok, t8);
#pragma unroll
          for (int e = 0; e < 8; ++e) xr[j][e] += t8[e];
        }
      }
    }
    const float* dsrc = static_cast<const float*>(a.dz) + (long)g * a.B * img_out + (long)b * img_out +
                        (long)h0 * W * NCBO * 8;
#pragma unroll
    for (int j = 0; j < DT; ++j) {
      const int i = tid + NT_ * j;
      if (i < DCH) load8f(dsrc + (long)i * 8, dr[j]);
    }
  };
  auto store = [&](int buf) {
#pragma unroll
    for (int j = 0; j < XT; ++j) {
      const int i = tid + NT_ * j;
      if (i < XCH) split8(xr[j], xs[buf][0][xslot(i)], xs[buf][1][xslot(i)], xs[buf][2][xslot(i)]);
    }
#pragma unroll
    for (int j = 0; j < DT; ++j) {
      const int i = tid + NT_ * j;
      if (i >= DCH) continue;
      uint4 q0, q1, q2;
      split8(dr[j], q0, q1, q2);
      ds[buf][0][dslot(i)] = q0;
      ds[buf][1][dslot(i)] = q1;
      ds[buf][2][dslot(i)] = q2;
      if (PK && i % NCBO == PKC) {
        const int creal = a.cout_real - 16 * (MT - 1);
        uint32_t w[8];
        const uint32_t h0[4] = {q0.x & 0xffffu, q0.x >> 16, q0.y & 0xffffu, q0.y >> 16};
        const uint32_t h1[4] = {q1.x & 0xffffu, q1.x >> 16, q1.y & 0xffffu, q1.y >> 16};
        const uint32_t h2[4] = {q2.x & 0xffffu, q2.x >> 16, q2.y & 0xffffu, q2.y >> 16};
#pragma unroll
        for (int c = 0; c < 4; ++c) {
          w[2 * c] = c < creal ? (h0[c] | (h1[c] << 16)) : 0u;
          w[2 * c + 1] = c < creal ? h2[c] : 0u;
        }
        const int px = i / NCBO;
        dpk[buf][px][0] = make_uint4(w[0], w[1], w[2], w[3]);
        dpk[buf][px][1] = make_uint4(w[4], w[5], w[6], w[7]);
      }
    }
  };

  const int gq = lane >> 4, q = (lane >> 2) & 3, p = lane & 3, l16 = lane & 15;
  const int px0 = 8 * gq + q;
  const int prow = px0 / W, pcol = px0 % W;
  const int xlane = (prow * PW + pcol) * XROW;
  const int dlane = px0 * DROW + p * 8;
  int xoff[TPW];
#pragma unroll
  for (int t = 0; t < TPW; ++t) {
    const int n = nz0 + wave + NW * t;
    int c = 2 * n + (p >> 1);
    if (c >= NCH) c = 0;
    const int kk = c / NCBI, cb = c % NCBI;
    xoff[t] = xlane + ((kk / KW) * PW + (kk % KW)) * XROW + cb * 16 + (p & 1) * 8;
  }
  const bool ones_lane = l16 == (NCH & 1) * 8;

  f32x4_t acc[MT][TPW];
#pragma unroll
  for (int m = 0; m < MT; ++m)
#pragma unroll
    for (int t = 0; t < TPW; ++t) acc[m][t] = (f32x4_t){0.f, 0.f, 0.f, 0.f};

  const bool early = NB == 2 && wave >= NW / 2;
  if (band0 < band1) {
    load(band0);
    store(0);
    if (early && band0 + 1 < band1) load(band0 + 1);
  }
  int cur = 0;
  for (int band = band0; band < band1; ++band, cur ^= (NB - 1)) {
    __syncthreads();
    const bool more = band + 1 < band1;
    if (early) {
      if (more) {
        store(cur ^ 1);
        if (band + 2 < band1) load(band + 2);
      }
    } else if (more) {
      load(band + 1);
    }
#pragma unroll
    for (int ks = 0; ks < KS; ++ks) {
      const int xrow_off = ((ks * 32) / W) * PW * XROW;
      auto load_at = [&](int m, uint4* af) {
        if (PK && m == MT - 1) {
          const char* d0 = reinterpret_cast<const char*>(dpk[cur]) + px0 * 32 + p * 8 + ks * 32 * 32;
          af[0] = tr_pair(d0, d0 + 4 * 32);
          return;
        }
#pragma unroll
        for (int pl = 0; pl < NPL; ++pl) {
          const char* d0 = reinterpret_cast<const char*>(ds[cur][pl]) + dlane + ks * 32 * DROW + m * 32;
          af[pl] = tr_pair(d0, d0 + 4 * DROW);
        }
      };
      auto load_bt = [&](int t, uint4* bfr) {
        const int n = nz0 + wave + NW * t;
#pragma unroll
        for (int pl = 0; pl < NPL; ++pl) {
          const char* x0 = reinterpret_cast<const char*>(xs[cur][pl]) + xrow_off + xoff[t];
          bfr[pl] = tr_pair(x0, x0 + 4 * XROW);
        }
        if (n == NCH / 2 && ones_lane) {
          bfr[0] = make_uint4(0x3f803f80u, 0x3f803f80u, 0x3f803f80u, 0x3f803f80u);
          bfr[1] = bfr[2] = make_uint4(0, 0, 0, 0);
        }
      };
      auto mma = [&](int m, const uint4* af, const uint4* bf, f32x4_t c) {
        if (PK && m == MT - 1) {
          c = mfma16(af[0], bf[2], c);
          c = mfma16(af[0], bf[1], c);
          return mfma16(af[0], bf[0], c);
        }
        return mfma_np<NPL>(af, bf, c);
      };
      if constexpr (MOUT) {
        uint4 bfr[TPW][NPL];
#pragma unroll
        for (int t = 0; t < TPW; ++t) load_bt(t, bfr[t]);
        uint4 af[2][NPL];
        load_at(0, af[0]);
#pragma unroll
        for (int m = 0; m < MT; ++m) {
          if (m + 1 < MT) load_at(m + 1, af[(m + 1) & 1]);
#pragma unroll
          for (int t = 0; t < TPW; ++t)
            if (nz0 + wave + NW * t < NKT) acc[m][t] = mma(m, af[m & 1], bfr[t], acc[m][t]);
        }
      } else {
        uint4 afr[MT][NPL];
#pragma unroll
        for (int m = 0; m < MT; ++m) load_at(m, afr[m]);
        uint4 bfr[2][NPL];
        load_bt(0, bfr[0]);
#pragma unroll
        for (int t = 0; t < TPW; ++t) {
          const int n = wave + NW * t;
          if (t + 1 < TPW) load_bt(t + 1, bfr[(t + 1) & 1]);
          if (n >= NKT) continue;
#pragma unroll
          for (int m = 0; m < MT; ++m) acc[m][t] = mma(m, afr[m], bfr[t & 1], acc[m][t]);
        }
      }
    }
    if (more && !early) {
      if (NB == 1) __syncthreads();
      store(cur ^ (NB - 1));
    }
  }

  const int kq = lane >> 4;
  constexpr int Kdim = NCH * 8;
#pragma unroll
  for (int t = 0; t < TPW; ++t) {
    const int n = nz0 + wave + NW * t;
    if (n >= NKT) continue;
    const int col = n * 16 + l16;
#pragma unroll
    for (int m = 0; m < MT; ++m)
#pragma unroll
      for (int i = 0; i < 4; ++i) {
        const bool pkm = PK && m == MT - 1;
        const int co = pkm ? m * 16 + kq + 4 * i : m * 16 + kq * 4 + i;
        const float v = pkm ? (i == 0 ? acc[m][t][0] + acc[m][t][1] + acc[m][t][2] : 0.f) : acc[m][t][i];
        if (co >= a.Coutp) continue;
        if (col < Kdim)
          a.part_w[(((long)s * a.G + g) * a.Coutp + co) * Kdim + col] = v;
        else if (col == Kdim && a.part_b)
          a.part_b[((long)s * a.G + g) * a.Coutp + co] = v;
      }
  }
}
```

### gentun_amd/models/cnn_hip.py

```python

import math

import numpy as np
import torch

from ..ops import cnn_kernels as K
from ..utils import rng as _rng
from .cnn_engine import FoldJob
from .pop_schedule import PopulationSchedule

WGRAD_STREAMS = 2
POOL_FUSE = True
NATIVE_STEPS = True

WINOGRAD = False

WFRAG = True

EVAL_TWIN_BUDGET = 1 << 30


def pad8(c):
    return (c + 7) // 8 * 8


def round_up(x, m):
    return (x + m - 1) // m * m


def split_planes(w, npl):
    out = torch.empty((npl,) + tuple(w.shape), dtype=torch.bfloat16, device=w.device)
    r = w.float()
    for q in range(npl):
        out[q] = r.to(torch.bfloat16)
        r = r - out[q].float()
    return out


def fast_path_report(plan, dtype="fp32", ngroups=25, B=32, pad_images=True, batch_norm=False):
    prec = K.PREC[dtype]
    h0r, w0r, c0 = plan.input_shape
    kernels, nodes = list(plan.kernels_per_layer), list(plan.nodes)
    ks = [tuple(k) for k in plan.kernel_sizes]
    hw = K.padded_hw(h0r, w0r, len(kernels), batch_norm)
    h0, w0 = hw if pad_images else (h0r, w0r)
    pads = K.stage_channel_pads(c0, kernels, ks, h0, w0, prec, ngroups=ngroups, B=B)
    lib = K.lib()
    layers, generic, fast = [], 0, 0
    cin, cinr = pad8(c0), c0
    for s, (cp, k) in enumerate(zip(pads, ks)):
        H, W = h0 >> s, w0 >> s
        for kind, (KH, KW), ci, cir, n in (("in", k, cin, cinr, 1), ("node/out", (3, 3), cp, kernels[s], nodes[s] + 1)):
            first = s == 0 and kind == "in"
            f = K.layer_fast(KH, KW, ci, cp, H, W, prec, ngroups, B, cir, kernels[s], first)
            wino = bool(WINOGRAD and prec == 1 and (KH, KW) == (3, 3) and lib.gt_conv_wino_supported(ci, cp, H, W)
                        and lib.gt_conv_wino_supported(cp, ci, H, W))
            nl = n * (2 if first else 3)
            bad = n * sum(1 for x in (f if not first else f[::2]) if not x)
            generic += bad
            fast += nl - bad
            layers.append({"stage": s, "layer": kind, "k": KH, "hw": H, "cin_p": ci, "cout_p": cp,
                           "fwd_fast": f[0], "dgrad_fast": None if first else f[1], "wgrad_fast": f[2],
                           "winograd": wino})
        cin, cinr = cp, kernels[s]
    return {"stored_hw": [h0, w0], "stage_channels_padded": pads, "fast_launches": fast,
            "generic_launches": generic, "layers": layers}


class HipPopJob(FoldJob):

    def __init__(self, plan, x, y, folds, cfg, device, **kw):
        if cfg.dtype not in K.PREC:
            raise ValueError("HIP backend precision must be one of {}".format(sorted(K.PREC)))
        self.layout = "nhwc8f" if cfg.dtype == "fp32" else "nhwc8"
        p0 = plan if plan is not None else kw["members"][0][0]
        h0r, w0r, _ = p0.input_shape
        hw = K.padded_hw(h0r, w0r, len(p0.kernels_per_layer), bool(getattr(cfg, "batch_norm", False)))
        self.pad_hw = hw if hw != (h0r, w0r) and getattr(cfg, "pad_images", True) else None
        super(HipPopJob, self).__init__(plan, x, y, folds, cfg, device, **kw)
        if self.device.type != "cuda":
            raise RuntimeError("the HIP backend needs a GPU device")
        self.L = K.lib()
        self.prec = K.PREC[cfg.dtype]
        self.npl = K.NPL[cfg.dtype]
        self.adt = torch.float32 if self.prec else torch.bfloat16
        self.bn = bool(getattr(cfg, "batch_norm", False))
        self._setup_dp()
        p0 = self.plan
        Q, B, dev = self.G, self.B, self.device
        self.Q = Q
        h0, w0, c0 = p0.input_shape
        if self.data.x.shape[-1] != pad8(c0):
            raise ValueError("dataset channels do not match the plan")
        self.classes = p0.classes
        if p0.classes > 16:
            raise ValueError("HIP head kernel supports at most 16 classes")
        if B > 64:
            raise ValueError("HIP head kernel supports batch_size <= 64")
        if max(p0.nodes) > K.MAXSLOT - 2:
            raise ValueError("at most {} nodes per stage".format(K.MAXSLOT - 2))
        self._build_topology()
        self._allocate()
        self.state = torch.zeros(8, dtype=torch.int32, device=dev)
        self.state_f = self.state.view(torch.float32)
        self.step_ctr = self.state[0:1]
        self.eval_state = torch.zeros(8, dtype=torch.int32, device=dev)
        self.fold_ids_t = torch.tensor(self.fold_ids, dtype=torch.int32, device=dev)
        seeds = [_rng.stable_hash(self.member_seeds[self.gmember[q]], "dropout") & 0xFFFFFFFF for q in range(Q)]
        self.drop_seeds_t = torch.tensor(np.asarray(seeds, np.uint32).view(np.int32), device=dev)
        self._keep = []
        ss = [torch.cuda.Stream(dev) for _ in range(WGRAD_STREAMS + 1)]
        self.wg_streams = ss[:WGRAD_STREAMS]
        self.side2 = ss[WGRAD_STREAMS]
        self.graph_streams = 2 + WGRAD_STREAMS
        self._build_adam_table()
        self._build_args()

    def _setup_dp(self):
        grp = getattr(self.cfg, "dp_group", None)
        self.dp = None
        if grp is None:
            return
        if self.bn:
            raise ValueError("data parallelism with BatchNorm would need synchronised batch statistics")
        import torch.distributed as dist
        world, rank = dist.get_world_size(grp), dist.get_rank(grp)
        B = self.B
        r0, r1 = rank * B // world, (rank + 1) * B // world
        if r1 <= r0:
            raise ValueError("data parallelism: batch {} over {} ranks leaves a rank without rows".format(B, world))
        self.dp = (grp, rank, world, r0, r1)
        self.capture_ok = False
        self.B_full = B
        self.epoch_idx_full = self.epoch_idx
        self.epoch_idx = torch.zeros((self.steps_per_epoch, self.G, r1 - r0), dtype=torch.int64, device=self.device)
        self.epoch_valid_full = self.epoch_valid
        self.epoch_valid = (self.epoch_valid_full - r0).clamp(0, r1 - r0).to(torch.int32).contiguous()
        self.B = r1 - r0

    def _new_epoch_order(self):
        if getattr(self, "dp", None) is None:
            return super(HipPopJob, self)._new_epoch_order()
        r0, r1 = self.dp[3], self.dp[4]
        local, self.epoch_idx, self.B = self.epoch_idx, self.epoch_idx_full, self.B_full
        try:
            super(HipPopJob, self)._new_epoch_order()
        finally:
            self.epoch_idx, self.B = local, r1 - r0
        self.epoch_idx.copy_(self.epoch_idx_full[:, :, r0:r1])

    def _dp_allreduce(self):
        import torch.distributed as dist
        grads = self._dp_grads
        flat = torch.cat([t.reshape(-1) for t in grads])
        if dist.get_backend(self.dp[0]) == "nccl":
            dist.all_reduce(flat, group=self.dp[0])
        else:
            host = flat.cpu()
            dist.all_reduce(host, group=self.dp[0])
            flat.copy_(host)
        o = 0
        for t in grads:
            n = t.numel()
            t.copy_(flat[o:o + n].view_as(t))
            o += n

    def _build_topology(self):
        p0, Q = self.plan, self.Q
        h0r, w0r, _ = p0.input_shape
        h0, w0 = self.pad_hw or (h0r, w0r)
        self.sched = PopulationSchedule([self.members[self.gmember[q]][0] for q in range(Q)], hw=self.pad_hw)
        self.stages, self.layers = self.sched.stages, self.sched.layers
        ks = [tuple(k) for k in p0.kernel_sizes]
        self.stage_cp = K.stage_channel_pads(p0.input_shape[2], list(p0.kernels_per_layer), ks, h0, w0,
                                             self.prec, ngroups=Q, B=self.B)
        for L in self.layers:
            L.coutp = self.stage_cp[L.stage]
            L.cinp = pad8(L.cin) if L.kind == "in" and L.stage == 0 else \
                self.stage_cp[L.stage - 1] if L.kind == "in" else L.coutp
            L.Kdim = L.KH * L.KW * L.cinp
            L.TH = K.conv_tile_rows(L.H, L.W)
            band = K.wgrad_band(L.KH, L.KW, L.cinp, L.coutp, L.H, L.W, self.prec)
            L.pps, L.S = K.wgrad_split(self.B * L.H * L.W, L.Kdim, L.coutp, band=band)
            L.wred = L.S > 1 and (L.coutp * L.Kdim) % 4 == 0
        self.last = self.sched.last
        hs, ws = h0 >> len(p0.kernels_per_layer), w0 >> len(p0.kernels_per_layer)
        if hs < 1 or ws < 1:
            raise ValueError("input too small for the pooling stages")
        self.final_hw = (hs, ws)
        self.final_hw_real = (h0r >> len(p0.kernels_per_layer), w0r >> len(p0.kernels_per_layer))
        self.final_cp = self.stage_cp[-1]

    def _allocate(self):
        Q, B, dev, p0 = self.Q, self.B, self.device, self.plan
        self.shapes = {}
        for st in self.stages:
            for L in st.layers:
                self.shapes[L.name] = (L.H, L.W, L.coutp)
            self.shapes[st.pool] = (st.H // 2, st.W // 2, self.stage_cp[st.s])
        self.act, self.grad = {}, {}
        for name, (hh, ww, cc) in self.shapes.items():
            self.act[name] = torch.zeros((Q, B, hh, ww, cc), dtype=self.adt, device=dev)
            self.grad[name] = torch.zeros((Q, B, hh, ww, cc), dtype=self.adt, device=dev)
        for L in self.layers:
            if L.xin is not None:
                self.act[L.xin] = torch.zeros((Q, B, L.H, L.W, L.cinp), dtype=self.adt, device=dev)
        self.zpre = {}
        if self.bn:
            for L in self.layers:
                self.zpre[L.name] = torch.zeros((Q, B, L.H, L.W, L.coutp), dtype=self.adt, device=dev)
                L.bn_chunk = K.bn_chunk_px(L.H, L.W, L.coutp)
                L.bn_nchunk = -(-(B * L.H * L.W) // L.bn_chunk)
                L.bn_stat = torch.zeros((Q, 2, L.coutp), dtype=torch.float32, device=dev)
                L.bn_run = torch.zeros((2, Q, L.coutp), dtype=torch.float32, device=dev)
                L.bn_part = torch.zeros((Q, L.bn_nchunk, 2, L.coutp), dtype=torch.float32, device=dev)
                L.g_gamma = torch.zeros((Q, L.coutp), dtype=torch.float32, device=dev)
                L.g_beta = torch.zeros((Q, L.coutp), dtype=torch.float32, device=dev)
        hs, ws = self.final_hw
        self.Fp = hs * ws * self.final_cp
        self.Up = round_up(p0.dense_units, 64)
        self.hdrop = torch.zeros((Q, B, self.Up), dtype=self.adt, device=dev)
        self.dH = torch.zeros((Q, B, self.Up), dtype=torch.float32, device=dev)
        self.dHp = torch.zeros((self.npl, Q, B, self.Up), dtype=torch.int16, device=dev)
        self.dz_head = torch.zeros((Q, B, self.classes), dtype=torch.float32, device=dev)
        self.plog = torch.zeros((Q, self.Up // 16, B, self.classes), dtype=torch.float32, device=dev)
        segs = []
        for L in self.layers:
            segs.append(("w", L, (Q, L.coutp, L.KH, L.KW, L.cinp)))
            segs.append(("b", L, (Q, L.coutp)))
            if self.bn:
                segs.append(("gamma", L, (Q, L.coutp)))
                segs.append(("beta", L, (Q, L.coutp)))
        segs.append(("W1", None, (Q, self.Fp, self.Up)))
        segs.append(("b1", None, (Q, self.Up)))
        segs.append(("W2", None, (Q, self.Up, self.classes)))
        segs.append(("b2", None, (Q, self.classes)))
        total = sum(int(np.prod(s)) for _, _, s in segs)
        self.flat = torch.zeros(total, dtype=torch.float32, device=dev)
        self.m = torch.zeros_like(self.flat)
        self.v = torch.zeros_like(self.flat)
        off = 0
        self.views = {}
        for kind, L, shape in segs:
            n = int(np.prod(shape))
            view = (self.flat[off:off + n].view(shape), self.m[off:off + n].view(shape),
                    self.v[off:off + n].view(shape))
            if L is not None:
                setattr(L, kind, view)
            else:
                self.views[kind] = view
            off += n
        npl = self.npl
        wsegs = []
        for L in self.layers:
            L.w_bf = torch.zeros((npl, Q, L.coutp, L.KH, L.KW, L.cinp), dtype=torch.bfloat16, device=dev)
            L.wT_bf = torch.zeros((npl, Q, L.cinp, L.KH, L.KW, L.coutp), dtype=torch.bfloat16, device=dev)
            L.wino = bool(WINOGRAD and self.prec == 1 and (L.KH, L.KW) == (3, 3) and
                          self.L.gt_conv_wino_supported(L.cinp, L.coutp, L.H, L.W) and
                          self.L.gt_conv_wino_supported(L.coutp, L.cinp, L.H, L.W))
            if L.wino:
                R, Kc = K.wino_dims(L.cinp, L.coutp)
                L.wU = torch.zeros((3, Q, 16, R, Kc), dtype=torch.bfloat16, device=dev)
                R, Kc = K.wino_dims(L.coutp, L.cinp)
                L.wUT = torch.zeros((3, Q, 16, R, Kc), dtype=torch.bfloat16, device=dev)
                wsegs += [K.wino_segment(L.w[0], L.wU, False), K.wino_segment(L.w[0], L.wUT, True)]
            L.part_w = torch.zeros((L.S, Q, L.coutp, L.Kdim), dtype=torch.float32, device=dev)
            L.part_b = torch.zeros((L.S, Q, L.coutp), dtype=torch.float32, device=dev)
        self.wino_tr = K.WinoTransform(wsegs, dev) if wsegs else None
        fspecs = []
        for L in self.layers:
            first = L.slots == ["input"]
            L.wfrag = L.wfragT = False
            if not WFRAG or L.wino:
                continue
            nr = max(1, len(L.rows))
            if K._probe_conv(self.L, L.KH, L.KW, L.cinp, L.coutp, L.H, L.W, self.prec, nr, B, L.cout, True):
                _, nks = K.frag_order(L.KH, L.KW, L.cinp // 8, L.W, self.prec)
                L.wF = torch.zeros((npl, Q, -(-L.coutp // 16) * nks * 512), dtype=torch.bfloat16, device=dev)
                fspecs.append((L.w[0], L.wF, L.W, self.prec, False))
                L.wfrag = True
            if not first and K._probe_conv(self.L, L.KH, L.KW, L.coutp, L.cinp, L.H, L.W, self.prec, nr, B, L.cin,
                                           False):
                _, nks = K.frag_order(L.KH, L.KW, L.coutp // 8, L.W, self.prec)
                L.wTF = torch.zeros((npl, Q, -(-L.cinp // 16) * nks * 512), dtype=torch.bfloat16, device=dev)
                fspecs.append((L.w[0], L.wTF, L.W, self.prec, True))
                L.wfragT = True
            L.bf_needed = not (L.wfrag and (L.wfragT or first))
        self.frag_tr = K.FragTransform(fspecs, dev) if fspecs else None
        self.gW2 = torch.zeros((Q, self.Up, self.classes), dtype=torch.float32, device=dev)
        self.gb2 = torch.zeros((Q, self.classes), dtype=torch.float32, device=dev)
        self.gb1 = torch.zeros((Q, self.Up), dtype=torch.float32, device=dev)

    def _gtab(self, rows):
        arr = np.zeros((max(1, len(rows)), 4), np.int32)
        for i, (g, im, of) in enumerate(rows):
            arr[i, 0], arr[i, 1], arr[i, 2] = g, im, of
        t = torch.from_numpy(arr).to(self.device)
        self._keep.append(t)
        return t

    def _build_adam_table(self):
        segs, blocks = [], []

        def add(p, m, v, g, S, gstride, bf=None, bfT=None, tdims=None, pstrides=(0, 0)):
            sg = K.AdamSeg()
            sg.p, sg.m, sg.v, sg.g = p.data_ptr(), m.data_ptr(), v.data_ptr(), g.data_ptr()
            sg.bf = bf.data_ptr() if bf is not None else 0
            sg.bfT = bfT.data_ptr() if bfT is not None else 0
            sg.npl = self.npl
            sg.pstride_bf, sg.pstride_bfT = pstrides
            sg.n = p.numel()
            sg.gstride = gstride
            sg.S = S
            ntiles = 0
            if tdims is not None:
                sg.tG, sg.tCo, sg.tKH, sg.tKW, sg.tCi = tdims
                ntiles = K.adam_tiles(*tdims) if bfT is not None else 0
            sg.tiled = 1 if ntiles else 0
            idx = len(segs)
            segs.append(sg)
            if ntiles:
                blocks.extend((idx, t) for t in range(ntiles))
            else:
                for o in K.adam_blocks(p.numel()):
                    blocks.append((idx, o))

        for L in self.layers:
            for q, _ in L.rows:
                p, m, v = (t[q] for t in L.w)
                S = 1 if L.wred else L.S
                if getattr(L, "bf_needed", True):
                    add(p, m, v, L.part_w[0, q], S, L.part_w[0].numel(), bf=L.w_bf[0, q], bfT=L.wT_bf[0, q],
                        tdims=(1, L.coutp, L.KH, L.KW, L.cinp), pstrides=(L.w_bf[0].numel(), L.wT_bf[0].numel()))
                else:
                    add(p, m, v, L.part_w[0, q], S, L.part_w[0].numel())
                p, m, v = (t[q] for t in L.b)
                add(p, m, v, L.part_b[0, q], S, L.part_b[0].numel())
                if self.bn:
                    for t, g in ((L.gamma, L.g_gamma), (L.beta, L.g_beta)):
                        p, m, v = (x[q] for x in t)
                        add(p, m, v, g[q], 1, g[q].numel())
        for name, g in (("b1", self.gb1), ("W2", self.gW2), ("b2", self.gb2)):
            p, m, v = self.views[name]
            add(p, m, v, g, 1, g.numel())
        arr = (K.AdamSeg * len(segs))(*segs)
        raw = bytes(memoryview(arr).cast("B"))
        self.adam_segs = torch.frombuffer(bytearray(raw), dtype=torch.uint8).to(self.device)
        self.adam_blocks = torch.tensor(np.asarray(blocks, np.int32).reshape(-1, 2), device=self.device)
        self.adam_nblocks = len(blocks)

    def _dense_sk_buffers(self, df, rows):
        nby, nut = -(-rows // 32), self.Up // 64
        part = torch.empty((self.Q * nby * nut * max(1, df.ks) * 4 * 2 * 64 * 4,), dtype=torch.float32,
                           device=self.device)
        self._keep.append(part)
        df.part, df.cnt = part.data_ptr(), 0

    def _conv_args(self, L, in_ptrs, out_ptrs, mask_ptrs, w, bias, relu, rows, gather=None, Cinp=None, Coutp=None):
        a = K.ConvArgs()
        for i, p in enumerate(in_ptrs):
            a.inp[i] = p
        for i, p in enumerate(out_ptrs):
            a.out[i] = p
        for i, p in enumerate(mask_ptrs):
            a.out_mask[i] = p
        a.relu = relu
        a.gather = gather or 0
        a.st = self.state.data_ptr()
        a.w = w.data_ptr()
        a.bias = bias.data_ptr() if bias is not None else 0
        a.gtab = self._gtab(rows).data_ptr()
        a.ngroups = len(rows)
        a.G, a.B, a.H, a.W = self.Q, self.B, L.H, L.W
        a.Cinp = L.cinp if Cinp is None else Cinp
        a.Coutp = L.coutp if Coutp is None else Coutp
        a.cout_real = L.cout if Coutp is None else L.cin
        a.KH, a.KW, a.TH = L.KH, L.KW, L.TH
        a.prec = self.prec
        a.wps = w[0].numel()
        return a

    def _bn_args(self, L, train, pools=()):
        a = K.BnArgs()
        a.z, a.y = self.zpre[L.name].data_ptr(), self.act[L.name].data_ptr()
        a.gamma, a.beta = L.gamma[0].data_ptr(), L.beta[0].data_ptr()
        a.stat, a.run, a.part = L.bn_stat.data_ptr(), L.bn_run.data_ptr(), L.bn_part.data_ptr()
        a.ggamma, a.gbeta = L.g_gamma.data_ptr(), L.g_beta.data_ptr()
        a.gtab = self._gtab([(q, 0, (1 << 24) if q in pools else 0) for q, _ in L.rows]).data_ptr()
        a.W = L.W
        a.valid = self.epoch_valid.data_ptr()
        a.st = self.state.data_ptr()
        a.ngroups, a.G, a.B, a.HW, a.Cp = len(L.rows), self.Q, self.B, L.H * L.W, L.coutp
        a.nchunk, a.chunk_px = L.bn_nchunk, L.bn_chunk
        a.momentum, a.eps = self.cfg.bn_momentum, self.cfg.bn_eps
        a.train, a.prec = train, self.prec
        if self.pad_hw is not None:
            a.Hr, a.Wr = L.Hr, L.Wr
        return a

    def _stage_fwd_ops(self, st, gather_train, fuse):
        src = self.sched.pool_source(st)
        x1 = self.sched.pool_x1(st)
        pool_of = {}
        if fuse:
            pool_of.setdefault(st.inp, set()).update(q for q in range(self.Q) if not src[q])
            pool_of.setdefault(x1, set()).update(q for q in range(self.Q) if src[q])
        ops = []
        for L in st.layers:
            first = L.slots == ["input"]
            out = self.zpre[L.name] if self.bn else self.act[L.name]
            pools = pool_of.get(L.name, set())
            cpools = set() if self.bn else pools
            a = self._conv_args(L, [self._slot_ptr(n) for n in L.slots], [out.data_ptr()], [],
                                L.wU if L.wino else L.wF if L.wfrag else L.w_bf, L.b[0], 0 if self.bn else 1,
                                [(q, im, 1 | ((1 << 24) if q in cpools else 0)) for q, im in L.rows],
                                gather=gather_train if first else None)
            a.wino = 1 if L.wino else 0
            a.wfrag = 1 if L.wfrag else 0
            if L.xin is not None:
                a.xsum = self.act[L.xin].data_ptr()
            if self.pad_hw is not None:
                a.Hr, a.Wr = L.Hr, L.Wr
            a.epi_bf16 = 1
            if cpools:
                a.pool_y, a.pool_mask = self.act[st.pool].data_ptr(), st.pmask.data_ptr()
            ops.append(("conv", a, L))
            if self.bn:
                b = self._bn_args(L, 1, pools)
                if pools:
                    b.pool_y, b.pool_mask = self.act[st.pool].data_ptr(), st.pmask.data_ptr()
                ops.append(("bn", b, L))
        return ops

    def _slot_ptr(self, name, grad=False):
        if name == "input":
            return self.data.x.data_ptr()
        t = (self.grad if grad else self.act).get(name)
        return t.data_ptr() if t is not None else 0

    def _build_args(self):
        Q, B = self.Q, self.B
        gather_train = self.epoch_idx.data_ptr()
        self.fwd_ops = []
        L_ = self.L
        fast_on = K.fast_path_on(L_)
        fuse_env = POOL_FUSE
        self.pool_fused = []
        for st in self.stages:
            hh, ww, cc = self.shapes[st.inp]
            fuse_ok = fuse_env and (K.BN_CHUNK_PX % (2 * ww) == 0 and hh % 2 == 0 if self.bn else fast_on)
            sel = torch.tensor(self.sched.pool_source(st), dtype=torch.int32, device=self.device)
            self._keep.append(sel)
            st.sel = sel
            st.pmask = torch.zeros((Q * B, hh // 2, ww // 2, cc), dtype=torch.uint8, device=self.device)
            ops = self._stage_fwd_ops(st, gather_train, fuse=fuse_ok)
            fused = fuse_ok and (self.bn or all(L_.gt_conv_fast_probe(a) > 0 for kind, a, _ in ops
                                                if kind == "conv" and a.pool_y))
            if not fused:
                ops = self._stage_fwd_ops(st, gather_train, fuse=False)
                x1 = self.act[self.sched.pool_x1(st)]
                ops.append(("pool", (self.act[st.inp].data_ptr(), x1.data_ptr(), sel.data_ptr(),
                                     self.act[st.pool].data_ptr(), Q * B, B, hh, ww, cc), st.pmask.data_ptr()))
            self.pool_fused.append(fused)
            self.fwd_ops.extend(ops)
        prec = self.prec
        df = K.DenseFwdArgs()
        df.x, df.wt, df.bias, df.out = (self.act[self.last].data_ptr(), 0, self.views["b1"][0].data_ptr(),
                                        self.hdrop.data_ptr())
        df.st, df.fold_ids, df.seeds = self.state.data_ptr(), self.fold_ids_t.data_ptr(), self.drop_seeds_t.data_ptr()
        df.G, df.B, df.Fp, df.Up = Q, B, self.Fp, self.Up
        df.drop_p, df.train, df.seed = self.cfg.dropout, 1, 0
        df.w2, df.plog, df.C = self.views["W2"][0].data_ptr(), self.plog.data_ptr(), self.classes
        df.prec, df.wps = prec, 0
        df.w1 = self.views["W1"][0].data_ptr()
        df.ks = int(self.L.gt_dense_fwd_splits(self.Fp))
        self._dense_sk_buffers(df, B)
        self.dense_fwd_args = df
        hd = K.HeadArgs()
        hd.h, hd.w2, hd.b2 = self.hdrop.data_ptr(), self.views["W2"][0].data_ptr(), self.views["b2"][0].data_ptr()
        hd.labels, hd.gather, hd.st = self.data.labels.data_ptr(), gather_train, self.state.data_ptr()
        hd.valid = self.epoch_valid.data_ptr()
        hd.dH, hd.gw2, hd.gb2, hd.gb1 = self.dH.data_ptr(), self.gW2.data_ptr(), self.gb2.data_ptr(), self.gb1.data_ptr()
        hd.eval_out = 0
        hd.dz = self.dz_head.data_ptr()
        hd.plog = self.plog.data_ptr()
        hd.G, hd.B, hd.Up, hd.C = Q, B, self.Up, self.classes
        hd.loss_ce = 1 if self.cfg.loss == "ce" else 0
        hd.drop_scale = 1.0 / (1.0 - self.cfg.dropout) if self.cfg.dropout < 1 else 0.0
        hd.eval = 0
        hd.prec = prec
        hd.dHp = self.dHp.data_ptr()
        self.head_args = hd
        dd = K.DenseDgradArgs()
        dd.dH, dd.wt, dd.dx = self.dH.data_ptr(), 0, self.grad[self.last].data_ptr()
        dd.dHp = self.dHp.data_ptr()
        dd.G, dd.B, dd.Fp, dd.Up = Q, B, self.Fp, self.Up
        dd.prec, dd.wps = prec, 0
        dd.w1 = self.views["W1"][0].data_ptr()
        self.dense_dgrad_args = dd
        dw = K.DenseWgradAdamArgs()
        p, m, v = self.views["W1"]
        dw.x, dw.dH, dw.p, dw.m, dw.v = self.act[self.last].data_ptr(), self.dH.data_ptr(), p.data_ptr(), \
            m.data_ptr(), v.data_ptr()
        dw.wt, dw.st = 0, self.state.data_ptr()
        dw.G, dw.B, dw.Fp, dw.Up = Q, B, self.Fp, self.Up
        dw.Cp, dw.Cr, dw.Ur = self.final_cp, self.plan.kernels_per_layer[-1], self.plan.dense_units
        dw.prec, dw.wps = prec, 0
        self.dense_wgrad_args = dw
        if self.dp is not None:
            self.gW1 = torch.zeros((Q, self.Fp, self.Up), dtype=torch.float32, device=self.device)
            dw.gbuf, dw.mode = self.gW1.data_ptr(), 1
            self.dense_apply_args = K.DenseWgradAdamArgs.from_buffer_copy(dw)
            self.dense_apply_args.mode = 2
            df.row_off = self.dp[3]
            hd.valid_norm = self.epoch_valid_full.data_ptr()
            self._dp_grads = [t for L in self.layers for t in (L.part_w[0], L.part_b[0])] + \
                [self.gW1, self.gW2, self.gb2, self.gb1]
        self.bwd_ops = []
        bn_done = set()
        fuse_bwd = fast_on and POOL_FUSE
        pool_stage = {st.pool: st for st in self.stages}
        self.unpool_fused = set()
        if fuse_bwd:
            st = self.stages[-1]
            hh, ww, cc = self.shapes[st.inp]
            dd.unpool_mask, dd.unpool_sel = st.pmask.data_ptr(), st.sel.data_ptr()
            dd.unpool_x0 = self.grad[st.inp].data_ptr()
            dd.unpool_x1 = self.grad[self.sched.pool_x1(st)].data_ptr()
            dd.Hs, dd.Ws, dd.Cp = hh, ww, cc
            self.unpool_fused.add(st.pool)
        for rec in self.sched.backward():
            if rec[0] == "pool_bwd":
                st = rec[1]
                if st.pool in self.unpool_fused:
                    continue
                hh, ww, cc = self.shapes[st.inp]
                x1 = self.sched.pool_x1(st)
                self.bwd_ops.append(("pool_bwd", (st.pmask.data_ptr(),
                                                  st.sel.data_ptr(), self.grad[st.pool].data_ptr(),
                                                  self.grad[st.inp].data_ptr(), self.grad[x1].data_ptr(),
                                                  Q * B, B, hh, ww, cc, 1, prec), None))
                continue
            kind, L, rows = rec
            first = L.slots == ["input"]
            if self.bn and L.name not in bn_done:
                bn_done.add(L.name)
                ba = self._bn_args(L, 1)
                ba.y = self.grad[L.name].data_ptr()
                self.bwd_ops.append(("bn_bwd", ba, L))
            if kind == "wgrad":
                wa = K.WgradArgs()
                wslots = L.slots + ([L.xin] if L.xin is not None else [])
                for i, n in enumerate(wslots):
                    wa.inp[i] = self._slot_ptr(n)
                wa.gather = gather_train if first else 0
                wa.st = self.state.data_ptr()
                wa.dz = self.grad[L.name].data_ptr()
                wa.part_w, wa.part_b = L.part_w.data_ptr(), L.part_b.data_ptr()
                wa.gtab = self._gtab([(q, im, 0) for q, im in rows]).data_ptr()
                wa.ngroups = len(rows)
                wa.G, wa.B, wa.H, wa.W = Q, B, L.H, L.W
                wa.Cinp, wa.Coutp, wa.KH, wa.KW, wa.S, wa.pps = L.cinp, L.coutp, L.KH, L.KW, L.S, L.pps
                wa.prec = prec
                wa.cout_real = L.cout
                self.bwd_ops.append(("wgrad", wa, L))
            else:
                def dgrad_args(unpool):
                    a = self._conv_args(L, [self.grad[L.name].data_ptr()],
                                        [self._slot_ptr(n, grad=True) for n in L.slots],
                                        [self._slot_ptr(n) for n in L.slots],
                                        L.wUT if L.wino else L.wTF if L.wfragT else L.wT_bf,
                                        None, 0, [(q, 1, of | ((1 << 25) if unpool else 0)) for q, of in rows],
                                        Cinp=L.coutp, Coutp=L.cinp)
                    a.wino = 1 if L.wino else 0
                    a.wfrag = 1 if L.wfragT else 0
                    if unpool:
                        st = pool_stage[L.slots[0]]
                        a.pool_y, a.pool_mask = self.grad[st.inp].data_ptr(), st.pmask.data_ptr()
                        a.unpool_x1 = self.grad[self.sched.pool_x1(st)].data_ptr()
                        a.unpool_sel = st.sel.data_ptr()
                    return a
                a = None
                if fuse_bwd and len(L.slots) == 1 and L.slots[0] in pool_stage:
                    a = dgrad_args(True)
                    if self.L.gt_conv_fast_probe_any(a):
                        self.unpool_fused.add(L.slots[0])
                    else:
                        a = None
                if a is None:
                    a = dgrad_args(False)
                self.bwd_ops.append(("conv", a, L))
        aa = K.AdamArgs()
        aa.segs, aa.blocks, aa.st = self.adam_segs.data_ptr(), self.adam_blocks.data_ptr(), self.state.data_ptr()
        self.adam_args = aa

    def _build_init_table(self):
        Q = self.Q
        segs, blocks, seeds = [], [], []

        def add(t, d, r, fan_in, fan_out, name):
            assert t.is_contiguous() and t.numel() == Q * int(np.prod(d))
            seeds.append([_rng.stable_hash(self._fold_seed(g), name) & 0x7FFFFFFFFFFFFFFF for g in range(Q)])
            sg = K.InitSeg()
            sg.p = t.data_ptr()
            for i in range(4):
                sg.d[i], sg.r[i] = int(d[i]), int(r[i])
            sg.G = Q
            sg.tag = _rng.stable_hash("tag", name) & 0x7FFFFFFF
            sg.limit = math.sqrt(6.0 / (fan_in + fan_out))
            idx = len(segs)
            segs.append(sg)
            for o in range(0, t.numel(), 256):
                blocks.append((idx, o))

        for L in self.layers:
            add(L.w[0], (L.coutp, L.KH, L.KW, L.cinp), (L.cout, L.KH, L.KW, L.cin), L.cin * L.KH * L.KW,
                L.cout * L.KH * L.KW, L.name + ".w")
        hs, ws = self.final_hw
        hr, wr = self.final_hw_real
        add(self.views["W1"][0], (hs, ws, self.final_cp, self.Up),
            (hr, wr, self.plan.kernels_per_layer[-1], self.plan.dense_units),
            self.plan.flatten, self.plan.dense_units, "dense1.w")
        w2 = self.views["W2"][0]
        add(w2, (1, 1, w2.shape[1], w2.shape[2]), (1, 1, self.plan.dense_units, self.plan.classes),
            self.plan.dense_units, self.plan.classes, "dense2.w")
        self.init_seeds = torch.tensor(np.asarray(seeds, np.int64), device=self.device)
        for k, sg in enumerate(segs):
            sg.seeds = self.init_seeds[k].data_ptr()
        arr = (K.InitSeg * len(segs))(*segs)
        self.init_segs = torch.frombuffer(bytearray(bytes(memoryview(arr).cast("B"))), dtype=torch.uint8
                                          ).to(self.device)
        self.init_blocks = torch.tensor(np.asarray(blocks, np.int32).reshape(-1, 2), device=self.device)
        ia = K.InitArgs()
        ia.segs, ia.blocks = self.init_segs.data_ptr(), self.init_blocks.data_ptr()
        self.init_args = ia
        self.init_nblocks = len(blocks)

    def init_params(self):
        if getattr(self, "init_args", None) is None:
            self._build_init_table()
        self.flat.zero_()
        K.check(K.lib().gt_glorot_init(self.init_args, self.init_nblocks, self._stream()), "glorot_init")
        if self.bn:
            for L in self.layers:
                L.gamma[0][:, :L.cout].fill_(1.0)
                L.bn_run[0].zero_()
                L.bn_run[1].fill_(1.0)
        self._refresh_copies()

    def _refresh_copies(self):
        for L in self.layers:
            w = L.w[0]
            L.w_bf.copy_(split_planes(w, self.npl))
            L.wT_bf.copy_(split_planes(w.flip(2, 3).permute(0, 4, 2, 3, 1), self.npl))
        if self.frag_tr is not None:
            self.frag_tr.run(self._stream())
        if self.wino_tr is not None:
            self.wino_tr.run(self._stream())

    def reset_optimizer(self, lr):
        self.m.zero_()
        self.v.zero_()
        self.state_f[2:3].zero_()
        self.state_f[3:4].fill_(float(lr))
        self.state[6:7].fill_(1 if self.cfg.optimizer == "sgd" else 0)
        self.state_f[7:8].fill_(float(self.cfg.momentum))

    def snapshot(self):
        return (self.flat.clone(), self.m.clone(), self.v.clone(), self.state.clone(),
                [L.bn_run.clone() for L in self.layers] if self.bn else [])

    @property
    def can_rebind(self):
        return self.dp is None

    def _rebind_device(self):
        self.fold_ids_t.copy_(torch.tensor(self.fold_ids, dtype=torch.int32))
        self.init_args = None
        self.state.zero_()
        self.eval_state.zero_()

    def copy_biases_from(self, other):
        mine = {L.name: L for L in self.layers}
        for L in other.layers:
            if L.name in mine:
                mine[L.name].b[0].copy_(L.b[0])
                if self.bn and other.bn:
                    mine[L.name].gamma[0].copy_(L.gamma[0])
                    mine[L.name].beta[0].copy_(L.beta[0])
                    mine[L.name].bn_run.copy_(L.bn_run)
        for name in ("b1", "b2"):
            self.views[name][0].copy_(other.views[name][0])

    def _kept_tensors(self):
        out = []
        for L in self.layers:
            out.append(L.b[0])
            if self.bn:
                out += [L.gamma[0], L.beta[0], L.bn_run]
        return out + [self.views["b1"][0], self.views["b2"][0]]

    def bias_state(self):
        return [t.clone() for t in self._kept_tensors()]

    def load_bias_state(self, state):
        for t, v in zip(self._kept_tensors(), state):
            t.copy_(v)
        self._refresh_copies()

    def restore(self, snap):
        self.flat.copy_(snap[0])
        self.m.copy_(snap[1])
        self.v.copy_(snap[2])
        self.state.copy_(snap[3])
        for L, r in zip(self.layers, snap[4]):
            L.bn_run.copy_(r)
        self._refresh_copies()

    def _stream(self):
        return torch.cuda.current_stream(self.device).cuda_stream

    def _run_fwd(self, s, ops):
        L = self.L
        for kind, a, mk in ops:
            if kind == "conv":
                K.check(L.gt_conv_fwd(a, s), "conv_fwd")
            elif kind == "bn":
                K.check(L.gt_bn_fwd(a, s), "bn_fwd")
            elif mk is not None:
                K.check(L.gt_pool_fwd_mask(*a, mk, self.prec, s), "pool_fwd")
            else:
                K.check(L.gt_pool_fwd(*a, self.prec, s), "pool_fwd")

    def _fwd_plan(self, ops):
        plan = []
        for kind, a, mk in ops:
            if kind == "conv":
                plan.append(("k", "gt_conv_fwd", (a,), None, "conv_fwd"))
            elif kind == "bn":
                plan.append(("k", "gt_bn_fwd", (a,), None, "bn_fwd"))
            elif mk is not None:
                plan.append(("k", "gt_pool_fwd_mask", tuple(a) + (mk, self.prec), None, "pool_fwd"))
            else:
                plan.append(("k", "gt_pool_fwd", tuple(a) + (self.prec,), None, "pool_fwd"))
        return plan

    def _step_plan(self):
        main = None
        plan = [("k", "gt_step_begin", (self.state.data_ptr(),), main, "step_begin")]
        plan += self._fwd_plan(self.fwd_ops)
        plan += [("k", "gt_dense_fwd", (self.dense_fwd_args,), main, "dense_fwd"),
                 ("k", "gt_head", (self.head_args,), main, "head"),
                 ("k", "gt_dense_dgrad", (self.dense_dgrad_args,), main, "dense_dgrad")]
        side2 = self.side2
        nev = [0]

        def edge(src, dst):
            if src is not dst:
                plan.append(("rec", src, nev[0]))
                plan.append(("wait", dst, nev[0]))
                nev[0] += 1

        edge(main, side2)
        plan.append(("k", "gt_dense_wgrad_adam", (self.dense_wgrad_args,), side2, "dense_wgrad_adam"))
        wgs = self.wg_streams
        nwg = 0
        for kind, a, Lr in self.bwd_ops:
            if kind == "wgrad":
                ws = wgs[nwg % len(wgs)]
                nwg += 1
                edge(main, ws)
                plan.append(("k", "gt_conv_wgrad", (a,), ws, "conv_wgrad"))
                if Lr.wred:
                    plan.append(("k", "gt_wgrad_reduce", (a,), ws, "wgrad_reduce"))
            elif kind == "conv":
                plan.append(("k", "gt_conv_fwd", (a,), main, "conv_dgrad"))
            elif kind == "bn_bwd":
                plan.append(("k", "gt_bn_bwd", (a,), main, "bn_bwd"))
            else:
                plan.append(("k", "gt_pool_bwd_mask", tuple(a), main, "pool_bwd"))
        for stream in [side2] + list(wgs):
            edge(stream, main)
        return plan

    def _adam_plan(self):
        plan = [("k", "gt_adam_segments", (self.adam_args, self.adam_nblocks), None, "adam")]
        if self.frag_tr is not None:
            plan.append(("k", "gt_conv_wfrag", (K.C.addressof(self.frag_tr.args), self.frag_tr.nblocks), None,
                         "conv_wfrag"))
        if self.wino_tr is not None:
            plan.append(("k", "gt_wino_wtrans", (K.C.addressof(self.wino_tr.args), self.wino_tr.nblocks), None,
                         "wino_wtrans"))
        return plan

    def _exec_plan(self, plan):
        L = self.L
        main = torch.cuda.current_stream(self.device)
        evs = {}
        for op in plan:
            st = op[3] if op[0] == "k" else op[1]
            st = main if st is None else st
            if op[0] == "k":
                K.check(getattr(L, op[1])(*op[2], st.cuda_stream), op[4])
            elif op[0] == "rec":
                ev = torch.cuda.Event()
                ev.record(st)
                evs[op[2]] = ev
            else:
                st.wait_event(evs[op[2]])

    def train_step(self):
        self._exec_plan(self._step_plan())
        if self.dp is not None:
            self._dp_allreduce()
            K.check(self.L.gt_dense_wgrad_adam(self.dense_apply_args, self._stream()), "dense_wgrad_adam(apply)")
        self._exec_plan(self._adam_plan())

    def train_steps(self, n):
        if self.dp is None and NATIVE_STEPS:
            prog = getattr(self, "_prog", None)
            if prog is None:
                prog = self._prog = K.StepProgram(self._step_plan() + self._adam_plan())
            prog.run(self._stream(), n)
            return
        for _ in range(n):
            self.train_step()

    def eval_batch(self):
        per_img = sum(t[0, 0].numel() * t.element_size() for t in self.act.values())
        per_img += sum(t[0, 0].numel() * t.element_size() for t in self.zpre.values())
        per_img += self.Up * 4 * 2
        maxv = int(self.val_mat.shape[1])
        eb = min(int(getattr(self.cfg, "eval_batch", 256) or 256), 256, round_up(maxv, 32))
        eb = min(eb, max(1, int(EVAL_TWIN_BUDGET // max(1, per_img * self.Q))) // 32 * 32)
        return max(self.B, eb)

    def _eval_ops(self, EB):
        cached = getattr(self, "_eval_cache", None)
        if cached is not None and cached[0] == EB:
            return cached[1]
        built = self._build_eval_ops(EB)
        self._eval_cache = (EB, built)
        return built

    def _build_eval_ops(self, EB):
        Q = self.Q
        remap, keep = {}, []

        def twin(t):
            e = torch.empty((Q, EB) + tuple(t.shape[2:]), dtype=t.dtype, device=t.device)
            remap[t.data_ptr()] = e.data_ptr()
            keep.append(e)
            return e
        for t in list(self.act.values()) + list(self.zpre.values()):
            twin(t)
        hdrop, plog = twin(self.hdrop), torch.empty((Q, self.Up // 16, EB, self.classes), dtype=torch.float32,
                                                    device=self.device)
        keep.append(plog)

        def rp(ptr):
            return remap.get(ptr, ptr)
        ops = []
        for kind, a, Lr in self.fwd_ops:
            if kind == "conv":
                b = K.ConvArgs.from_buffer_copy(a)
                for i in range(K.MAXSLOT):
                    b.inp[i], b.out[i] = rp(b.inp[i] or 0), rp(b.out[i] or 0)
                b.st = self.eval_state.data_ptr()
                b.xsum = 0
                b.pool_y = rp(b.pool_y or 0)
                b.pool_mask = 0
                b.B = EB
                ops.append((kind, b, Lr))
            elif kind == "bn":
                b = K.BnArgs.from_buffer_copy(a)
                b.z, b.y, b.pool_y = rp(b.z or 0), rp(b.y or 0), rp(b.pool_y or 0)
                b.train = 0
                b.pool_mask = 0
                b.B = EB
                b.nchunk = -(-(EB * b.HW) // b.chunk_px)
                ops.append((kind, b, Lr))
            else:
                xin, x1, sel, py, _qb, _b, hh, ww, cc = a
                ops.append((kind, (rp(xin), rp(x1), sel, rp(py), Q * EB, EB, hh, ww, cc), None))
        df = K.DenseFwdArgs.from_buffer_copy(self.dense_fwd_args)
        df.x, df.out, df.plog = rp(df.x), hdrop.data_ptr(), plog.data_ptr()
        df.B, df.train = EB, 0
        self._dense_sk_buffers(df, EB)
        hd = K.HeadArgs.from_buffer_copy(self.head_args)
        hd.h, hd.plog = hdrop.data_ptr(), plog.data_ptr()
        hd.B, hd.eval, hd.st = EB, 1, self.eval_state.data_ptr()
        return ops, df, hd, keep

    def evaluate(self):
        Q, dev = self.Q, self.device
        EB = self.eval_batch()
        maxv = self.val_mat.shape[1]
        nch = -(-maxv // EB)
        idx = torch.zeros((Q, nch * EB), dtype=torch.int64, device=dev)
        mask = torch.zeros((Q, nch * EB), dtype=torch.float32, device=dev)
        idx[:, :maxv] = self.val_mat
        mask[:, :maxv] = self.val_mask
        table = idx.view(Q, nch, EB).permute(1, 0, 2).contiguous()
        out = torch.zeros((nch, Q, EB, 3), dtype=torch.float32, device=dev)
        ops, df, hd, keep = self._eval_ops(EB)
        self._eval_keep = (table, out, keep)
        s = self._stream()
        L = self.L
        for c in range(nch):
            gptr = table[c].data_ptr()
            for kind, b, _ in ops:
                if kind == "conv" and b.gather:
                    b.gather = gptr
            self._run_fwd(s, ops)
            K.check(L.gt_dense_fwd(df, s), "dense_fwd(eval)")
            hd.gather, hd.eval_out = gptr, out[c].data_ptr()
            K.check(L.gt_head(hd, s), "head(eval)")
        res = out.permute(1, 0, 2, 3).reshape(Q, nch * EB, 3) * mask[:, :, None]
        sums = res.double().sum(1).float()
        return sums[:, 0], sums[:, 1], sums[:, 2]


HipFoldJob = HipPopJob
```

### gentun_amd/ops/cnn_kernels.py

```python

import ctypes as C
import os

from . import _lib

P = C.c_void_p
I = C.c_int


MAXSLOT = 8

PREC = {"bf16": 0, "fp32": 1}
NPL = {"bf16": 1, "fp32": 3}


class GroupRec(C.Structure):
    _fields_ = [("g", I), ("in_mask", I), ("out_mask", I), ("pad", I)]


class ConvArgs(C.Structure):
    _fields_ = [("inp", P * MAXSLOT), ("mask", P), ("gather", P), ("st", P), ("out", P * MAXSLOT),
                ("out_mask", P * MAXSLOT), ("w", P), ("bias", P), ("gtab", P),
                ("n_in", I), ("n_out", I), ("acc_flags", I), ("relu", I),
                ("G", I), ("B", I), ("H", I), ("W", I), ("Cinp", I), ("Coutp", I), ("KH", I), ("KW", I),
                ("TH", I), ("ngroups", I), ("xsum", P), ("dbg", I), ("epi_bf16", I), ("prec", I), ("wps", C.c_long),
                ("cbb", I), ("pool_y", P), ("pool_mask", P), ("unpool_x1", P), ("unpool_sel", P),
                ("cout_real", I), ("Hr", I), ("Wr", I), ("wino", I), ("wfrag", I)]


class WinoWSeg(C.Structure):
    _fields_ = [("w", P), ("u", P), ("ups", C.c_long), ("Q", I), ("Cop", I), ("Cip", I), ("R", I), ("K", I),
                ("dgrad", I), ("pad", I)]


class WinoWArgs(C.Structure):
    _fields_ = [("segs", P), ("blocks", P)]


class FragSeg(C.Structure):
    _fields_ = [("w", P), ("dst", P), ("order", P), ("ps", C.c_long), ("Q", I), ("Cop", I), ("Cip", I), ("KH", I),
                ("KW", I), ("NT", I), ("NKS", I), ("NCBIc", I), ("dgrad", I), ("npl", I)]


class FragArgs(C.Structure):
    _fields_ = [("segs", P), ("blocks", P)]


def frag_order(KH, KW, ncbi, W, prec):
    nks = (KH * KW * ncbi + 3) // 4
    out = (C.c_int * (nks * 4))()
    lib().gt_conv_frag_order(KH, KW, ncbi, W, prec, out, nks * 4)
    return list(out), nks


class FragTransform(object):

    def __init__(self, specs, device):
        import numpy as np
        import torch
        segs, blocks, self._keep = [], [], []
        for master, planes, W, prec, dgrad in specs:
            Q, cop, KH, KW, cip = master.shape
            ncbi = (cop if dgrad else cip) // 8
            nt = -(-(cip if dgrad else cop) // 16)
            order, nks = frag_order(KH, KW, ncbi, W, prec)
            assert tuple(planes.shape) == (planes.shape[0], Q, nt * nks * 512) and planes.is_contiguous()
            ot = torch.tensor(order, dtype=torch.int32, device=device)
            self._keep.append(ot)
            sg = FragSeg()
            sg.w, sg.dst, sg.order, sg.ps = master.data_ptr(), planes.data_ptr(), ot.data_ptr(), planes[0].numel()
            sg.Q, sg.Cop, sg.Cip, sg.KH, sg.KW = Q, cop, cip, KH, KW
            sg.NT, sg.NKS, sg.NCBIc, sg.dgrad, sg.npl = nt, nks, ncbi, 1 if dgrad else 0, planes.shape[0]
            n = Q * nt * nks * 64
            blocks.extend((len(segs), o) for o in range(0, n, 256))
            segs.append(sg)
        arr = (FragSeg * max(1, len(segs)))(*segs)
        self.segs_t = torch.frombuffer(bytearray(bytes(memoryview(arr).cast("B"))), dtype=torch.uint8).to(device)
        self.blocks_t = torch.tensor(np.asarray(blocks, np.int32).reshape(-1, 2), device=device)
        self.args = FragArgs()
        self.args.segs, self.args.blocks = self.segs_t.data_ptr(), self.blocks_t.data_ptr()
        self.nblocks = len(blocks)

    def run(self, stream):
        if self.nblocks:
            check(lib().gt_conv_wfrag(C.addressof(self.args), self.nblocks, stream), "conv_wfrag")


def frag_planes(master, W, prec=1, dgrad=False):
    import torch
    Q, cop, KH, KW, cip = master.shape
    nt = -(-(cip if dgrad else cop) // 16)
    _, nks = frag_order(KH, KW, (cop if dgrad else cip) // 8, W, prec)
    planes = torch.zeros((3 if prec else 1, Q, nt * nks * 512), dtype=torch.bfloat16, device=master.device)
    tr = FragTransform([(master.contiguous(), planes, W, prec, dgrad)], master.device)
    tr.run(torch.cuda.current_stream(master.device).cuda_stream)
    return planes


def wino_dims(cinp, coutp):
    return -(-coutp // 16) * 16, -(-cinp // 32) * 32


class WgradArgs(C.Structure):
    _fields_ = [("inp", P * MAXSLOT), ("gather", P), ("st", P), ("dz", P), ("part_w", P),
                ("part_b", P), ("gtab", P), ("n_in", I), ("G", I), ("B", I), ("H", I), ("W", I), ("Cinp", I),
                ("Coutp", I), ("KH", I), ("KW", I), ("S", I), ("pps", I), ("ngroups", I), ("prec", I),
                ("cout_real", I)]


class ConvSel(C.Structure):
    _fields_ = [(n, I) for n in ("KH", "KW", "NCBI", "W", "TH", "NT", "NCO", "NWV", "PREC", "PK", "RE", "CTX", "SCH",
                                 "lds_fwd", "lds_bwd", "gx", "gy", "gz", "block", "lds")]


class WgradSel(C.Structure):
    _fields_ = [(n, I) for n in ("KH", "KW", "NCBI", "NCBO", "W", "R", "NW", "NB", "PK", "NZ", "PREC",
                                 "gx", "gy", "gz", "block", "lds")]


class DenseFwdArgs(C.Structure):
    _fields_ = [("x", P), ("wt", P), ("bias", P), ("out", P), ("w2", P), ("plog", P), ("st", P), ("fold_ids", P),
                ("seeds", P), ("G", I), ("B", I), ("Fp", I), ("Up", I), ("drop_p", C.c_float), ("train", I),
                ("seed", C.c_uint), ("C", I), ("prec", I), ("wps", C.c_long), ("row_off", I),
                ("w1", P), ("part", P), ("cnt", P), ("ks", I)]


class HeadArgs(C.Structure):
    _fields_ = [("h", P), ("w2", P), ("b2", P), ("labels", P), ("gather", P), ("st", P), ("dH", P),
                ("gw2", P), ("gb2", P), ("gb1", P), ("eval_out", P), ("dz", P), ("plog", P),
                ("G", I), ("B", I), ("Up", I), ("C", I), ("loss_ce", I), ("drop_scale", C.c_float), ("eval", I),
                ("prec", I), ("valid", P), ("valid_norm", P), ("dHp", P)]


class DenseDgradArgs(C.Structure):
    _fields_ = [("dH", P), ("wt", P), ("dx", P), ("G", I), ("B", I), ("Fp", I), ("Up", I), ("prec", I),
                ("wps", C.c_long), ("unpool_mask", P), ("unpool_x0", P), ("unpool_x1", P), ("unpool_sel", P),
                ("Hs", I), ("Ws", I), ("Cp", I), ("w1", P), ("dHp", P)]


class DenseWgradAdamArgs(C.Structure):
    _fields_ = [("x", P), ("dH", P), ("p", P), ("m", P), ("v", P), ("wt", P), ("st", P),
                ("G", I), ("B", I), ("Fp", I), ("Up", I), ("Cp", I), ("Cr", I), ("Ur", I), ("prec", I),
                ("wps", C.c_long), ("gbuf", P), ("mode", I)]


class AdamSeg(C.Structure):
    _fields_ = [("p", P), ("m", P), ("v", P), ("g", P), ("bf", P), ("bfT", P), ("n", C.c_long),
                ("gstride", C.c_long), ("S", I), ("tG", I), ("tCo", I), ("tKH", I), ("tKW", I), ("tCi", I),
                ("tiled", I), ("npl", I), ("pstride_bf", C.c_long), ("pstride_bfT", C.c_long)]

ADAM_TK = 64


ADAM_BLK = 1024


def adam_blocks(n):
    return range(0, n, ADAM_BLK)


def adam_tiles(tG, tCo, tKH, tKW, tCi):
    if tCo % 8:
        return 0
    kd = tKH * tKW * tCi
    return tG * (-(-tCo // 128)) * (-(-kd // ADAM_TK))


class BnArgs(C.Structure):
    _fields_ = [("z", P), ("y", P), ("gamma", P), ("beta", P), ("stat", P), ("run", P), ("part", P),
                ("ggamma", P), ("gbeta", P), ("gtab", P), ("valid", P), ("st", P),
                ("ngroups", I), ("G", I), ("B", I), ("HW", I), ("Cp", I), ("nchunk", I), ("chunk_px", I),
                ("momentum", C.c_float), ("eps", C.c_float), ("train", I), ("prec", I),
                ("pool_y", P), ("pool_mask", P), ("W", I), ("Hr", I), ("Wr", I)]


BN_CHUNK_PX = 512
BN_CHUNK_VALUES = 16384


def bn_chunk_px(H, W, Cp):
    c = BN_CHUNK_PX
    pooled = BN_CHUNK_PX % (2 * W) == 0
    while c * Cp > BN_CHUNK_VALUES and (c // 2 >= 2 * W and (c // 2) % (2 * W) == 0 if pooled else c > 64):
        c //= 2
    return c


class AdamArgs(C.Structure):
    _fields_ = [("segs", P), ("blocks", P), ("st", P)]


class ProgOp(C.Structure):
    _fields_ = [("kind", C.c_int32), ("stream", C.c_int32), ("event", C.c_int32), ("pad", C.c_int32),
                ("v", C.c_int64 * 14)]


PROG_OPS = {"record": 0, "wait": 1, "gt_step_begin": 2, "gt_conv_fwd": 3, "gt_conv_wgrad": 4,
            "gt_wgrad_reduce": 5, "gt_bn_fwd": 6, "gt_bn_bwd": 7, "gt_dense_fwd": 8, "gt_head": 9,
            "gt_dense_dgrad": 10, "gt_dense_wgrad_adam": 11, "gt_adam_segments": 12, "gt_pool_fwd": 13,
            "gt_pool_fwd_mask": 14, "gt_pool_bwd_mask": 15, "gt_wino_wtrans": 16,
            "gt_conv_wfrag": 17}


class InitSeg(C.Structure):
    _fields_ = [("p", P), ("seeds", P), ("d", I * 4), ("r", I * 4), ("G", I), ("tag", I), ("limit", C.c_float),
                ("pad", I)]


class InitArgs(C.Structure):
    _fields_ = [("segs", P), ("blocks", P)]


_TYPED = {}


def lib():
    L = _lib.hip()
    if not _TYPED.get(id(L)):
        for name, argt in (("gt_conv_fwd", C.POINTER(ConvArgs)), ("gt_conv_wgrad", C.POINTER(WgradArgs)),
                           ("gt_dense_fwd", C.POINTER(DenseFwdArgs)), ("gt_head", C.POINTER(HeadArgs)),
                           ("gt_dense_dgrad", C.POINTER(DenseDgradArgs)),
                           ("gt_dense_wgrad_adam", C.POINTER(DenseWgradAdamArgs))):
            fn = getattr(L, name)
            fn.argtypes = [argt, P]
            fn.restype = I
        for name in ("gt_bn_fwd", "gt_bn_bwd"):
            fn = getattr(L, name)
            fn.argtypes = [C.POINTER(BnArgs), P]
            fn.restype = I
        L.gt_adam_segments.argtypes = [C.POINTER(AdamArgs), I, P]
        L.gt_adam_segments.restype = I
        L.gt_step_begin.argtypes = [P, P]
        L.gt_step_begin.restype = I
        L.gt_pool_fwd.argtypes = [P, P, P, P, I, I, I, I, I, I, P]
        L.gt_pool_fwd.restype = I
        L.gt_pool_bwd.argtypes = [P, P, P, P, P, P, I, I, I, I, I, I, I, P]
        L.gt_pool_bwd.restype = I
        L.gt_pool_fwd_mask.argtypes = [P, P, P, P, I, I, I, I, I, P, I, P]
        L.gt_pool_fwd_mask.restype = I
        L.gt_pool_bwd_mask.argtypes = [P, P, P, P, P, I, I, I, I, I, I, I, P]
        L.gt_pool_bwd_mask.restype = I
        L.gt_wgrad_set_nb.argtypes = [I]
        L.gt_wgrad_set_nb.restype = I
        L.gt_wgrad_fast_band.argtypes = [I, I, I, I, I, I, I]
        L.gt_wgrad_fast_splits.argtypes = [I, I, I, I, I, I, I]
        L.gt_wgrad_fast_splits.restype = I
        L.gt_wgrad_fast_band.restype = I
        L.gt_conv_fast_probe.argtypes = [C.POINTER(ConvArgs)]
        L.gt_conv_fast_probe.restype = I
        L.gt_conv_fast_probe_any.argtypes = [C.POINTER(ConvArgs)]
        L.gt_conv_fast_probe_any.restype = I
        L.gt_conv_fast_select.argtypes = [C.POINTER(ConvArgs), C.POINTER(ConvSel)]
        L.gt_conv_fast_select.restype = I
        L.gt_wgrad_fast_select.argtypes = [C.POINTER(WgradArgs), C.POINTER(WgradSel)]
        L.gt_wgrad_fast_select.restype = I
        L.gt_sizeof_conv_sel.restype = C.c_size_t
        assert L.gt_sizeof_conv_sel() == C.sizeof(ConvSel), "ConvSel ABI mismatch"
        L.gt_sizeof_wgrad_sel.restype = C.c_size_t
        assert L.gt_sizeof_wgrad_sel() == C.sizeof(WgradSel), "WgradSel ABI mismatch"
        L.gt_wgrad_reduce.argtypes = [C.POINTER(WgradArgs), P]
        L.gt_wgrad_reduce.restype = I
        L.gt_conv_frag_order.argtypes = [I, I, I, I, I, C.POINTER(C.c_int), I]
        L.gt_conv_frag_order.restype = I
        L.gt_conv_wfrag.argtypes = [P, I, P]
        L.gt_conv_wfrag.restype = I
        L.gt_sizeof_frag_seg.restype = C.c_size_t
        assert L.gt_sizeof_frag_seg() == C.sizeof(FragSeg), "FragSeg ABI mismatch"
        L.gt_conv_wino_supported.argtypes = [I, I, I, I]
        L.gt_conv_wino_supported.restype = I
        L.gt_wino_wtrans.argtypes = [P, I, P]
        L.gt_wino_wtrans.restype = I
        L.gt_sizeof_wino_wseg.restype = C.c_size_t
        assert L.gt_sizeof_wino_wseg() == C.sizeof(WinoWSeg), "WinoWSeg ABI mismatch"
        L.gt_conv_set_fast.argtypes = [I]
        L.gt_conv_set_fast.restype = I
        L.gt_dense_fwd_splits.argtypes = [I]
        L.gt_dense_fwd_splits.restype = I
        L.gt_conv_set_smallq.argtypes = [I]
        L.gt_conv_set_smallq.restype = I
        L.gt_conv_set_s2in_ct1.argtypes = [I]
        L.gt_conv_set_s2in_ct1.restype = I
        L.gt_conv_set_imgs.argtypes = [I]
        L.gt_conv_set_imgs.restype = I
        L.gt_glorot_init.argtypes = [C.POINTER(InitArgs), I, P]
        L.gt_glorot_init.restype = I
        L.gt_glorot_ref.argtypes = [C.c_uint64, C.c_uint64, I, C.c_float]
        L.gt_glorot_ref.restype = C.c_float
        L.gt_prog_create.argtypes = [C.POINTER(ProgOp), I, I, I]
        L.gt_prog_create.restype = P
        L.gt_prog_run.argtypes = [P, P, I, C.POINTER(I)]
        L.gt_prog_run.restype = I
        L.gt_prog_destroy.argtypes = [P]
        L.gt_prog_destroy.restype = None
        L.gt_sizeof_prog_op.restype = C.c_size_t
        assert L.gt_sizeof_prog_op() == C.sizeof(ProgOp), "ProgOp ABI mismatch"
        for name in ("gt_sizeof_conv_args", "gt_sizeof_wgrad_args", "gt_sizeof_adam_seg", "gt_sizeof_init_seg",
                     "gt_sizeof_dense_fwd_args", "gt_sizeof_head_args", "gt_sizeof_dense_dgrad_args",
                     "gt_sizeof_dense_wgrad_args", "gt_sizeof_bn_args"):
            getattr(L, name).restype = C.c_size_t
        assert L.gt_sizeof_conv_args() == C.sizeof(ConvArgs), "ConvArgs ABI mismatch"
        assert L.gt_sizeof_init_seg() == C.sizeof(InitSeg), "InitSeg ABI mismatch"
        assert L.gt_sizeof_wgrad_args() == C.sizeof(WgradArgs), "WgradArgs ABI mismatch"
        assert L.gt_sizeof_adam_seg() == C.sizeof(AdamSeg), "AdamSeg ABI mismatch"
        assert L.gt_adam_block_elems() == ADAM_BLK, "Adam block size mismatch"
        assert L.gt_sizeof_bn_args() == C.sizeof(BnArgs), "BnArgs ABI mismatch"
        for nm, st in (("dense_fwd_args", DenseFwdArgs), ("head_args", HeadArgs),
                       ("dense_dgrad_args", DenseDgradArgs), ("dense_wgrad_args", DenseWgradAdamArgs)):
            assert getattr(L, "gt_sizeof_" + nm)() == C.sizeof(st), nm + " ABI mismatch"
        _TYPED[id(L)] = True
    return L


def check(rc, what):
    if rc != 0:
        raise RuntimeError("HIP kernel launch {} failed with code {}".format(what, rc))


class StepProgram(object):

    def __init__(self, plan):
        L = lib()
        self.L = L
        keys, nev = [None], 0
        ops = (ProgOp * len(plan))()
        for o, op in zip(ops, plan):
            st = op[3] if op[0] == "k" else op[1]
            if not any(st is k for k in keys):
                keys.append(st)
            o.stream = next(i for i, k in enumerate(keys) if k is st)
            if op[0] in ("rec", "wait"):
                o.kind = PROG_OPS["record" if op[0] == "rec" else "wait"]
                o.event = int(op[2])
                nev = max(nev, o.event + 1)
                continue
            o.kind = PROG_OPS[op[1]]
            vals = []
            for a in op[2]:
                if isinstance(a, C.Structure):
                    vals.append(C.addressof(a))
                elif a is None:
                    vals.append(0)
                elif isinstance(a, C.c_void_p):
                    vals.append(a.value or 0)
                else:
                    vals.append(int(a))
            if len(vals) > len(o.v):
                raise ValueError("step program: too many operands for " + op[1])
            for i, x in enumerate(vals):
                o.v[i] = x
        self._ops = ops
        self._structs = [a for op in plan if op[0] == "k" for a in op[2] if isinstance(a, C.Structure)]
        self.keys = keys
        self.h = L.gt_prog_create(ops, len(plan), nev, len(keys))
        if not self.h:
            raise RuntimeError("gt_prog_create rejected the step program")
        self._streams = (C.c_void_p * len(keys))()

    def run(self, main_stream, nsteps):
        self._streams[0] = main_stream
        for i, k in enumerate(self.keys[1:], 1):
            self._streams[i] = k.cuda_stream
        bad = I(-1)
        rc = self.L.gt_prog_run(self.h, self._streams, int(nsteps), C.byref(bad))
        if rc != 0:
            raise RuntimeError("HIP step program op {} failed with code {}".format(bad.value, rc))

    def __del__(self):
        h, self.h = getattr(self, "h", None), None
        if h:
            try:
                self.L.gt_prog_destroy(h)
            except Exception:
                pass


def ptr(t):
    return C.c_void_p(t.data_ptr()) if t is not None else C.c_void_p(0)


CONV_TILE_PIXELS = 128


def conv_tile_rows(H, W, tile_pixels=None):
    tp = tile_pixels or CONV_TILE_PIXELS
    if W > tp:
        raise ValueError("image width > {} not supported by conv_fwd tiles".format(tp))
    return max(1, min(H, tp // W))


def wino_segment(master, planes, dgrad):
    Q, cop, kh, kw, cip = master.shape
    assert (kh, kw) == (3, 3) and master.dtype.is_floating_point and master.is_contiguous()
    R, Kc = (wino_dims(cop, cip) if dgrad else wino_dims(cip, cop))
    assert tuple(planes.shape) == (3, Q, 16, R, Kc) and planes.is_contiguous(), (planes.shape, (3, Q, 16, R, Kc))
    sg = WinoWSeg()
    sg.w, sg.u, sg.ups = master.data_ptr(), planes.data_ptr(), planes[0].numel()
    sg.Q, sg.Cop, sg.Cip, sg.R, sg.K, sg.dgrad = Q, cop, cip, R, Kc, 1 if dgrad else 0
    return sg


class WinoTransform(object):

    def __init__(self, segs, device):
        import numpy as np
        import torch
        self.nseg = len(segs)
        blocks = []
        for i, sg in enumerate(segs):
            n = sg.Q * sg.R * sg.K
            blocks.extend((i, o) for o in range(0, n, 256))
        arr = (WinoWSeg * max(1, len(segs)))(*segs)
        self.segs_t = torch.frombuffer(bytearray(bytes(memoryview(arr).cast("B"))), dtype=torch.uint8).to(device)
        self.blocks_t = torch.tensor(np.asarray(blocks, np.int32).reshape(-1, 2), device=device)
        self.args = WinoWArgs()
        self.args.segs, self.args.blocks = self.segs_t.data_ptr(), self.blocks_t.data_ptr()
        self.nblocks = len(blocks)

    def run(self, stream):
        if self.nblocks:
            check(lib().gt_wino_wtrans(C.addressof(self.args), self.nblocks, stream), "wino_wtrans")


def wino_unpack(planes):
    npl, Q, nxi, R, Kc = planes.shape
    f = planes.reshape(npl, Q, nxi, R // 16, Kc // 32, 4, 16, 8)
    return f.permute(0, 1, 2, 3, 6, 4, 5, 7).reshape(npl, Q, nxi, R, Kc)


def wino_weights(master, dgrad=False, stream=None):
    import torch
    Q, cop, _, _, cip = master.shape
    R, Kc = wino_dims(cop, cip) if dgrad else wino_dims(cip, cop)
    planes = torch.zeros((3, Q, 16, R, Kc), dtype=torch.bfloat16, device=master.device)
    tr = WinoTransform([wino_segment(master.contiguous(), planes, dgrad)], master.device)
    tr.run(torch.cuda.current_stream(master.device).cuda_stream if stream is None else stream)
    tr.keep = planes
    return planes


def padded_hw(h, w, nstages, batch_norm=False):
    del batch_norm
    p = 1 << max(0, int(w) - 1).bit_length()
    if (h != w or p == w or p > 1.25 * w or w % (1 << nstages) or p >> nstages < 8):
        return h, w
    return p, p


FAST_PADS = (24, 32, 56, 64, 104, 128, 256)


def fast_path_on(L):
    on = L.gt_conv_set_fast(1)
    L.gt_conv_set_fast(on)
    return bool(on)


def _probe_conv(L, KH, KW, cinp, coutp, H, W, prec, ngroups, B, cout_real, fwd):
    a = ConvArgs()
    a.KH, a.KW, a.Cinp, a.Coutp, a.H, a.W = KH, KW, cinp, coutp, H, W
    a.G = a.ngroups = max(1, ngroups)
    a.B, a.prec, a.cout_real = B, prec, cout_real
    a.epi_bf16 = 1 if fwd else 0
    a.TH = conv_tile_rows(H, W)
    return bool(L.gt_conv_fast_probe_any(a))


def layer_fast(KH, KW, cinp, coutp, H, W, prec, ngroups, B, cin_real, cout_real, first):
    L = lib()
    if not fast_path_on(L):
        return False, False, False
    fwd = _probe_conv(L, KH, KW, cinp, coutp, H, W, prec, ngroups, B, cout_real, True)
    dgr = True if first else _probe_conv(L, KH, KW, coutp, cinp, H, W, prec, ngroups, B, cin_real, False)
    wgr = int(L.gt_wgrad_fast_band(KH, KW, cinp, coutp, H, W, prec)) > 0
    return fwd, dgr, wgr


def stage_channel_pads(c0, kernels, kernel_sizes, h0, w0, prec, ngroups=25, B=32, max_factor=2.0):
    import itertools
    c0p = (c0 + 7) // 8 * 8
    base = [(c + 7) // 8 * 8 for c in kernels]
    cands = [sorted({b} | {v for v in FAST_PADS if b <= v <= max_factor * b}) for b in base]
    best = None
    for combo in itertools.product(*cands):
        cost, ok = 0.0, True
        cin, cinr = c0p, c0
        for s, (cp, k) in enumerate(zip(combo, kernel_sizes)):
            H, W = h0 >> s, w0 >> s
            kh, kw = tuple(k)
            for (KH, KW, ci, cir, first) in ((kh, kw, cin, cinr, s == 0), (3, 3, cp, kernels[s], False)):
                f = layer_fast(KH, KW, ci, cp, H, W, prec, ngroups, B, cir, kernels[s], first)
                if not all(f):
                    ok = False
                    break
                cost += H * W * KH * KW * ci * cp
            if not ok:
                break
            cin, cinr = cp, kernels[s]
        if ok and (best is None or cost < best[0]):
            best = (cost, combo)
    return list(best[1]) if best is not None else base


def wgrad_blocks(kdim, with_bias=True):
    return -(-(kdim + (8 if with_bias else 0)) // 64)


WGRAD_TARGET_BLOCKS = 50
WGRAD_FAST_SPLITS = 0


def wgrad_band(KH, KW, cinp, coutp, H, W, prec=0):
    L = lib()
    if not fast_path_on(L):
        return 0, 0
    band = int(L.gt_wgrad_fast_band(KH, KW, cinp, coutp, H, W, prec))
    splits = int(L.gt_wgrad_fast_splits(KH, KW, cinp, coutp, H, W, prec)) if band else 0
    return band, splits


def wgrad_split(npix, kdim, coutp, G=None, target_blocks=None, band=0):
    band, splits = band if isinstance(band, tuple) else (band, 8)
    if band:
        splits = WGRAD_FAST_SPLITS or splits
        nb = npix // band
        bps = -(-nb // max(1, splits))
        return bps * band, -(-nb // bps)
    if target_blocks is None:
        target_blocks = WGRAD_TARGET_BLOCKS
    nb = wgrad_blocks(kdim)
    mb = -(-coutp // 64)
    per = max(1, nb * mb)
    S = max(1, min(target_blocks // per, npix // 128))
    pps = -(-npix // S)
    pps = max(64, -(-pps // 64) * 64)
    S = -(-npix // pps)
    return pps, S
```

Before: 1056.

## Add two-pass patch staging for 3x3 Cin=56 fp32 conv to cut LDS footprint

Adds a two-pass variant of the fast conv kernel for one shape (3x3, 7 channel blocks, W=16, fp32). The input patch is staged in two channel halves that share a smaller LDS buffer, with the k-steps of the first half computed before the second half is staged. The variant also raises waves-per-EU from 2 to 3 and splits B-fragment loads into half batches to lower register pressure. This adds extra barriers and a serialized second staging phase in exchange for higher occupancy, and enables it by default through a Python flag plus a host query.

```diff
diff --git a/csrc/hip/cnn_args.h b/csrc/hip/cnn_args.h
--- a/csrc/hip/cnn_args.h
+++ b/csrc/hip/cnn_args.h
@@ -43,6 +43,7 @@
   int Hr, Wr;
   int wino;
   int wfrag;
+  int twopass;
 };
 
 __device__ __forceinline__ GroupRec group_rec(const GroupRec* gtab, int y, int n_in, int n_out, int acc,
diff --git a/csrc/hip/cnn_conv_fast.hip b/csrc/hip/cnn_conv_fast.hip
--- a/csrc/hip/cnn_conv_fast.hip
+++ b/csrc/hip/cnn_conv_fast.hip
@@ -33,7 +33,8 @@
     {8, 4, {tile<3, 3, 3, 32, 4, 2, 3, 2, 1, 1>(IF_TH | IF_PK), tile<3, 3, 3, 32, 4, 2, 3, 2, 1>(IF_TH),
             tile<3, 3, 3, 32, 8, 2, 3, 4, 1, 1>(IF_PK), tile<3, 3, 3, 32, 8, 2, 3, 4, 1>()}},
     {8, 2, {tile<5, 5, 3, 16, 4, 4, 7, 4, 1>(IF_TH), ct1<5, 5, 3, 16, 2, 4, 7, 4>(IF_TH), ct1<5, 5, 3, 16, 8, 4, 7, 4, 0>()}},
-    {8, 2, {tile<3, 3, 7, 16, 4, 4, 7, 4, 1>(IF_TH), ct1<3, 3, 7, 16, 2, 4, 7, 4>(IF_TH), ct1<3, 3, 7, 16, 8, 4, 7, 4, 0>()}},
+    {8, 2, {tile<3, 3, 7, 16, 4, 4, 7, 4, 1>(IF_TH), ct1<3, 3, 7, 16, 2, 4, 7, 4>(IF_TH),
+            ct1<3, 3, 7, 16, 8, 4, 7, 4, 0, 1>(IF_TWO), ct1<3, 3, 7, 16, 8, 4, 7, 4, 0>()}},
     {8, 4, {ct1<5, 5, 7, 16, 4, 2, 3, 4>(IF_S2CT1 | IF_TH), ct1<5, 5, 7, 16, 8, 2, 3, 4>(IF_S2CT1),
             tile<5, 5, 7, 16, 8, 2, 3, 4, 1, 1>(IF_PK), tile<5, 5, 7, 16, 8, 2, 3, 4, 1>()}},
     {8, 8, {tile<5, 5, 7, 8, 8, 7, 13, 7, 1>()}},
@@ -68,7 +69,8 @@
 
 static bool variant_ok(const ConvArgs* a, const ConvRow& r, const ConvVariant& v) {
   return (!(v.cond & IF_TH) || smallq_th(a, r.hmod, r.thmin) == v.k.TH) && (!(v.cond & IF_PK) || pk_ok(a, v.k.NT)) &&
-         (!(v.cond & IF_RE) || g_fast.regepi) && (!(v.cond & IF_S2CT1) || g_fast.s2in_ct1);
+         (!(v.cond & IF_RE) || g_fast.regepi) && (!(v.cond & IF_S2CT1) || g_fast.s2in_ct1) &&
+         (!(v.cond & IF_TWO) || a->twopass);
 }
 
 static bool select_conv(const ConvArgs* a, ConvChoice* c) {
@@ -136,6 +138,21 @@
   return 1;
 }
 extern "C" size_t gt_sizeof_conv_sel() { return sizeof(ConvSel); }
+
+extern "C" int gt_conv_fast_twopass(const ConvArgs* a) {
+  ConvChoice c;
+  if (a->wino || (a->prec != 0 && a->prec != 1) || !select_conv(a, &c)) return -1;
+  return c.k->TWO;
+}
+
+extern "C" int gt_conv_fast_occupancy(const ConvArgs* a) {
+  ConvChoice c;
+  int n = 0;
+  if (a->wino || (a->prec != 0 && a->prec != 1) || !select_conv(a, &c)) return -1;
+  lds_limit(c.k->fn, c.lds);
+  if (hipOccupancyMaxActiveBlocksPerMultiprocessor(&n, c.k->fn, (int)c.block, c.lds) != hipSuccess) return -1;
+  return n;
+}
 
 __global__ void __launch_bounds__(256) wgrad_reduce_kernel(WgradArgs a) {
   const GroupRec gr = group_rec(a.gtab, blockIdx.y, a.n_in, 0, 0, nullptr);
diff --git a/csrc/hip/conv_fast_host.h b/csrc/hip/conv_fast_host.h
--- a/csrc/hip/conv_fast_host.h
+++ b/csrc/hip/conv_fast_host.h
@@ -17,16 +17,17 @@
 struct ConvKernel {
   int KH, KW, NCBI, W, TH, NT, NCO, NWV, PREC, PK, RE, CTX, SCH;
   int lds_fwd, lds_bwd;
+  int TWO;
   const void* fn;
 };
 
 template <int KH, int KW, int NCBI, int W, int TH, int NT, int NCO, int NWV, int PREC, int PK = 0, int RE = 0,
-          int CTX = 0, int SCH = 0>
+          int CTX = 0, int SCH = 0, int TWO = 0>
 static ConvKernel conv_kernel() {
   static_assert((NCO * 8 + 15) / 16 == NT, "NT co tiles of 16 cover the NCO chunks of 8 channels");
-  using Cfg = FastCfg<KH, KW, NCBI, W, TH, NT, NCO, PREC>;
-  return {KH, KW, NCBI, W, TH, NT, NCO, NWV, PREC, PK, RE, CTX, SCH, (int)Cfg::lds(true), (int)Cfg::lds(false),
-          reinterpret_cast<const void*>(&conv_fast_kernel<KH, KW, NCBI, W, TH, NT, NCO, NWV, PREC, PK, RE, CTX, SCH>)};
+  using Cfg = FastCfg<KH, KW, NCBI, W, TH, NT, NCO, PREC, TWO>;
+  return {KH, KW, NCBI, W, TH, NT, NCO, NWV, PREC, PK, RE, CTX, SCH, (int)Cfg::lds(true), (int)Cfg::lds(false), TWO,
+          reinterpret_cast<const void*>(&conv_fast_kernel<KH, KW, NCBI, W, TH, NT, NCO, NWV, PREC, PK, RE, CTX, SCH, TWO>)};
 }
 
 enum : int {
@@ -34,6 +35,7 @@
   IF_PK = 2,
   IF_RE = 4,
   IF_S2CT1 = 8,
+  IF_TWO = 16,
 };
 
 struct ConvVariant {
@@ -50,9 +52,9 @@
   return v;
 }
 
-template <int KH, int KW, int NCBI, int W, int TH, int NT, int NCO, int NWV, int SCH = 1>
+template <int KH, int KW, int NCBI, int W, int TH, int NT, int NCO, int NWV, int SCH = 1, int TWO = 0>
 static ConvVariants ct1(int cond = 0) {
-  return {{cond, conv_kernel<KH, KW, NCBI, W, TH, NT, NCO, NWV, 1, 0, 1, 1, SCH>()}};
+  return {{cond, conv_kernel<KH, KW, NCBI, W, TH, NT, NCO, NWV, 1, 0, 1, 1, SCH, TWO>()}};
 }
 
 struct ConvRow {
diff --git a/csrc/hip/conv_fast_impl.h b/csrc/hip/conv_fast_impl.h
--- a/csrc/hip/conv_fast_impl.h
+++ b/csrc/hip/conv_fast_impl.h
@@ -19,9 +19,13 @@
   static constexpr int e0 = KH * KW * 4;
 };
 
-template <int KH, int KW, int NCBI, int W, int TH, int NT, int NCO, int PREC>
+template <int KH, int KW, int NCBI, int W, int TH, int NT, int NCO, int PREC, int TWO = 0>
 struct FastCfg {
+  static_assert(!TWO || S2Parts<KH, KW, NCBI, W, PREC>::on, "two-pass staging follows the part-major order");
   static constexpr int NPL = PREC ? GT_NPL_F32 : 1;
+  static constexpr int NC0 = TWO ? 4 : NCBI;
+  static constexpr int NC1 = NCBI - NC0;
+  static constexpr int NCL = NC0 > NC1 ? NC0 : NC1;
   static constexpr int PW = W + KW - 1;
   static constexpr int NP = (TH + KH - 1) * PW * NCBI;
   static constexpr int NCBP = NCBI + ((NCBI & 1) ? 0 : 1);
@@ -36,9 +40,10 @@
   static constexpr long LDS_PM = (long)NPIX * NCBP * 16 * NPL_ > OTILE ? (long)NPIX * NCBP * 16 * NPL_ : OTILE;
   static constexpr long LDS_PR = (long)((NCBI + 1) / 2) * PP2 * 16 * NPL_ > OTILE ? (long)((NCBI + 1) / 2) * PP2 * 16 * NPL_ : OTILE;
   static constexpr long LDS_CU = 160 * 1024;
-  static constexpr bool PAIR = PREC == 1 && NCBI >= 2 && LDS_CU / LDS_PR >= LDS_CU / LDS_PM;
+  static constexpr bool PAIR = TWO || (PREC == 1 && NCBI >= 2 && LDS_CU / LDS_PR >= LDS_CU / LDS_PM);
   static constexpr int PXS = PAIR ? 2 : NCBP;
-  static constexpr int NPP = PAIR ? ((NCBI + 1) / 2) * PP2 : NPIX * NCBP;
+  static constexpr int NPP = PAIR ? ((NCL + 1) / 2) * PP2 : NPIX * NCBP;
+  __host__ __device__ static constexpr int cloc(int cb) { return cb < NC0 ? cb : cb - NC0; }
   __host__ __device__ static constexpr int cbo(int cb) { return PAIR ? (cb >> 1) * PP2 + (cb & 1) : cb; }
   static size_t lds(bool fwd) {
     const size_t p = (size_t)NPP * 16 * NPL;
@@ -104,24 +109,18 @@
                                              const f32x4_t (&acc)[CT][PG], int wco, int pgw, int lane);
 
 template <int KH, int KW, int NCBI, int W, int TH, int NT, int NCO, int NWV = 4, int PREC = 0, int PK = 0, int RE = 0,
-          int CTX = 0, int SCH = 0>
+          int CTX = 0, int SCH = 0, int TWO = 0>
 __global__ void __launch_bounds__(NWV * 64)
-__attribute__((amdgpu_waves_per_eu(PREC ? 2 : (NWV == 8 ? 4 : (NT >= 4 ? (NCBI >= 7 ? 2 : 3) : 4)))))
+__attribute__((amdgpu_waves_per_eu(PREC ? (TWO ? 3 : 2) : (NWV == 8 ? 4 : (NT >= 4 ? (NCBI >= 7 ? 2 : 3) : 4)))))
 conv_fast_kernel(ConvArgs a) {
   typedef typename ActT<PREC>::T AT;
   constexpr int NPL = PREC ? GT_NPL_F32 : 1;
   constexpr int NTH = NWV * 64;
   constexpr int PH = TH + KH - 1, PW = W + KW - 1;
-  constexpr int NP = PH * PW * NCBI;
-  using FCL = FastCfg<KH, KW, NCBI, W, TH, NT, NCO, PREC>;
+  using FCL = FastCfg<KH, KW, NCBI, W, TH, NT, NCO, PREC, TWO>;
   constexpr int NCBP = FCL::NCBP;
   constexpr int PXS = FCL::PXS;
   constexpr int NPP = FCL::NPP;
-  auto pslot = [&](int i) {
-    if constexpr (NCBP == NCBI && !FCL::PAIR) return i;
-    else return (i / NCBI) * PXS + FCL::cbo(i % NCBI);
-  };
-  constexpr int NPT = (NP + NTH - 1) / NTH;
   constexpr int NCH = KH * KW * NCBI;
   constexpr int NKS = (NCH + 3) / 4;
   constexpr bool PARTS = S2Parts<KH, KW, NCBI, W, PREC>::on;
@@ -140,7 +139,7 @@
   constexpr int WC = NT / CT;
   constexpr int WP = NWV / WC;
   constexpr int PG = NPG / WP;
-  constexpr int PFM = PREC ? ((CTX == 1 && !SCH && NWV == 4 && NCBI <= 7) ? 3 : 2) : 4;
+  constexpr int PFM = PREC ? ((CTX == 1 && !SCH && NWV == 4 && NCBI <= 7 && !TWO) ? 3 : 2) : 4;
   constexpr int PF = NKS < PFM ? NKS : PFM;
   constexpr bool SCHED = SCH && PREC != 0 && NKS <= 64;
   constexpr int RA = SCHED ? PF + 1 : PF;
@@ -148,7 +147,7 @@
   static_assert(!PK || (PREC == 1 && WC == 1), "packed last tile: fp32, every wave owns all co tiles");
   static_assert(W % 16 == 0 || 16 % W == 0, "pixel groups must tile image rows");
 
-  using FC = FastCfg<KH, KW, NCBI, W, TH, NT, NCO, PREC>;
+  using FC = FCL;
   constexpr int OROW = FC::OROW, OROWB = FC::OROWB;
   extern __shared__ __attribute__((aligned(16))) uint4 smem[];
   uint4* patch = smem;
@@ -217,113 +216,124 @@
   const int n_src = a.gather ? 1 : __builtin_popcount(gr.in_mask);
   const AT* src0 = a.gather ? static_cast<const AT*>(a.in[0]) + a.gather[((long)a.st->cur_step * a.G + g) * a.B + b] * img
                             : static_cast<const AT*>(a.in[__builtin_ctz(gr.in_mask | 0x100) & 7]) + gimg;
-  long poff[NPT];
-  bool pok[NPT];
-#pragma unroll
-  for (int j = 0; j < NPT; ++j) {
-    const int i = tid + NTH * j;
-    const int cb = i % NCBI, pix = i / NCBI;
-    const int pr = pix / PW, pc = pix % PW;
-    const int hh = h0 - KH / 2 + pr, ww = pc - KW / 2;
-    pok[j] = i < NP && hh >= 0 && hh < a.H && ww >= 0 && ww < W;
-    poff[j] = ((long)hh * W + ww) * (NCBI * 8) + cb * 8;
-  }
-  if (a.dbg & 4) {
-#pragma unroll
-    for (int j = 0; j < NPT; ++j)
-#pragma unroll
-      for (int p = 0; p < NPL; ++p)
-        if (tid + NTH * j < NP) patch[p * NPP + pslot(tid + NTH * j)] = make_uint4(0, 0, 0, 0);
-  } else if (!PREC && n_src == 1) {
-    uint4 v[NPT];
-#pragma unroll
-    for (int j = 0; j < NPT; ++j)
-      v[j] = *reinterpret_cast<const uint4*>(pok[j] ? (const void*)(src0 + poff[j]) : (const void*)gt_zero8);
-#pragma unroll
-    for (int j = 0; j < NPT; ++j)
-      if (tid + NTH * j < NP) patch[pslot(tid + NTH * j)] = v[j];
-  } else {
-    constexpr int JB = NPT < 5 ? NPT : 5;
-#pragma unroll
-    for (int j0 = 0; j0 < NPT; j0 += JB) {
-      float acc8[JB][8];
-#pragma unroll
-      for (int j = 0; j < JB; ++j)
-#pragma unroll
-        for (int e = 0; e < 8; ++e) acc8[j][e] = 0.f;
-      if (n_src == 1) {
+  auto stage = [&](auto cb0_, auto nc_) {
+    constexpr int CB0 = decltype(cb0_)::value, NC = decltype(nc_)::value;
+    constexpr int NP = PH * PW * NC;
+    constexpr int NPT = (NP + NTH - 1) / NTH;
+    auto pslot = [&](int i) {
+      if constexpr (NCBP == NCBI && !FCL::PAIR) return i;
+      else return (i / NC) * PXS + FCL::cbo(i % NC);
+    };
+    long poff[NPT];
+    bool pok[NPT];
+#pragma unroll
+    for (int j = 0; j < NPT; ++j) {
+      const int i = tid + NTH * j;
+      const int cb = CB0 + i % NC, pix = i / NC;
+      const int pr = pix / PW, pc = pix % PW;
+      const int hh = h0 - KH / 2 + pr, ww = pc - KW / 2;
+      pok[j] = i < NP && hh >= 0 && hh < a.H && ww >= 0 && ww < W;
+      poff[j] = ((long)hh * W + ww) * (NCBI * 8) + cb * 8;
+    }
+    if (a.dbg & 4) {
+#pragma unroll
+      for (int j = 0; j < NPT; ++j)
+#pragma unroll
+        for (int p = 0; p < NPL; ++p)
+          if (tid + NTH * j < NP) patch[p * NPP + pslot(tid + NTH * j)] = make_uint4(0, 0, 0, 0);
+    } else if (!PREC && n_src == 1) {
+      uint4 v[NPT];
+#pragma unroll
+      for (int j = 0; j < NPT; ++j)
+        v[j] = *reinterpret_cast<const uint4*>(pok[j] ? (const void*)(src0 + poff[j]) : (const void*)gt_zero8);
+#pragma unroll
+      for (int j = 0; j < NPT; ++j)
+        if (tid + NTH * j < NP) patch[pslot(tid + NTH * j)] = v[j];
+    } else {
+      constexpr int JB = NPT < 5 ? NPT : 5;
+#pragma unroll
+      for (int j0 = 0; j0 < NPT; j0 += JB) {
+        float acc8[JB][8];
 #pragma unroll
         for (int j = 0; j < JB; ++j)
-          if (j0 + j < NPT && pok[j0 + j]) ld_chunk(src0 + poff[j0 + j], acc8[j]);
-      } else {
-        int m = gr.in_mask & 0xff;
-        while (m) {
-          const int k0 = __builtin_ctz(m);
-          m &= m - 1;
-          const bool two = m != 0;
-          const int k1 = two ? __builtin_ctz(m) : k0;
-          if (two) m &= m - 1;
-          const AT* s0 = static_cast<const AT*>(a.in[k0]) + gimg;
-          const AT* s1 = static_cast<const AT*>(a.in[k1]) + gimg;
-          float t0[JB][8], t1[JB][8];
-#pragma unroll
-          for (int j = 0; j < JB; ++j) {
-#pragma unroll
-            for (int e = 0; e < 8; ++e) t0[j][e] = t1[j][e] = 0.f;
-            if (j0 + j < NPT && pok[j0 + j]) {
-              ld_chunk(s0 + poff[j0 + j], t0[j]);
-              if (two) ld_chunk(s1 + poff[j0 + j], t1[j]);
+#pragma unroll
+          for (int e = 0; e < 8; ++e) acc8[j][e] = 0.f;
+        if (n_src == 1) {
+#pragma unroll
+          for (int j = 0; j < JB; ++j)
+            if (j0 + j < NPT && pok[j0 + j]) ld_chunk(src0 + poff[j0 + j], acc8[j]);
+        } else {
+          int m = gr.in_mask & 0xff;
+          while (m) {
+            const int k0 = __builtin_ctz(m);
+            m &= m - 1;
+            const bool two = m != 0;
+            const int k1 = two ? __builtin_ctz(m) : k0;
+            if (two) m &= m - 1;
+            const AT* s0 = static_cast<const AT*>(a.in[k0]) + gimg;
+            const AT* s1 = static_cast<const AT*>(a.in[k1]) + gimg;
+            float t0[JB][8], t1[JB][8];
+#pragma unroll
+            for (int j = 0; j < JB; ++j) {
+#pragma unroll
+              for (int e = 0; e < 8; ++e) t0[j][e] = t1[j][e] = 0.f;
+              if (j0 + j < NPT && pok[j0 + j]) {
+                ld_chunk(s0 + poff[j0 + j], t0[j]);
+                if (two) ld_chunk(s1 + poff[j0 + j], t1[j]);
+              }
+            }
+#pragma unroll
+            for (int j = 0; j < JB; ++j)
+#pragma unroll
+              for (int e = 0; e < 8; ++e) acc8[j][e] += t0[j][e];
+            if (two) {
+#pragma unroll
+              for (int j = 0; j < JB; ++j)
+#pragma unroll
+                for (int e = 0; e < 8; ++e) acc8[j][e] += t1[j][e];
             }
           }
-#pragma unroll
-          for (int j = 0; j < JB; ++j)
-#pragma unroll
-            for (int e = 0; e < 8; ++e) acc8[j][e] += t0[j][e];
-          if (two) {
-#pragma unroll
-            for (int j = 0; j < JB; ++j)
-#pragma unroll
-              for (int e = 0; e < 8; ++e) acc8[j][e] += t1[j][e];
+        }
+#pragma unroll
+        for (int j = 0; j < JB; ++j) {
+          const int i = tid + NTH * (j0 + j);
+          if (j0 + j >= NPT || i >= NP) continue;
+          if (PREC) {
+            uint4 p0, p1, p2;
+            split8(acc8[j], p0, p1, p2);
+            patch[pslot(i)] = p0;
+            patch[NPP + pslot(i)] = p1;
+            patch[2 * NPP + pslot(i)] = p2;
+          } else {
+            patch[pslot(i)] = pack8(acc8[j]);
           }
         }
       }
-#pragma unroll
-      for (int j = 0; j < JB; ++j) {
-        const int i = tid + NTH * (j0 + j);
-        if (j0 + j >= NPT || i >= NP) continue;
+    }
+    if (a.xsum && n_src > 1) {
+      __syncthreads();
+      AT* xo = static_cast<AT*>(a.xsum) + ((long)g * a.B + b) * img + (long)h0 * W * NCBI * 8;
+      for (int i = tid; i < TH * W * NC; i += NTH) {
+        const int cl = i % NC, pix = i / NC;
+        const int r = pix / W, c = pix % W;
+        if (h0 + r >= a.H) continue;
+        const int pi = ((r + KH / 2) * PW + c + KW / 2) * PXS + FCL::cbo(cl);
+        const long o = NC == NCBI ? (long)i * 8 : ((long)pix * NCBI + CB0 + cl) * 8;
         if (PREC) {
-          uint4 p0, p1, p2;
-          split8(acc8[j], p0, p1, p2);
-          patch[pslot(i)] = p0;
-          patch[NPP + pslot(i)] = p1;
-          patch[2 * NPP + pslot(i)] = p2;
+          float f[8];
+          join8(patch[pi], patch[NPP + pi], patch[2 * NPP + pi], f);
+          st_chunk(xo + o, f);
         } else {
-          patch[pslot(i)] = pack8(acc8[j]);
-        }
-      }
-    }
-  }
-  if (a.xsum && n_src > 1) {
-    __syncthreads();
-    AT* xo = static_cast<AT*>(a.xsum) + ((long)g * a.B + b) * img + (long)h0 * W * NCBI * 8;
-    for (int i = tid; i < TH * W * NCBI; i += NTH) {
-      const int cb = i % NCBI, pix = i / NCBI;
-      const int r = pix / W, c = pix % W;
-      if (h0 + r >= a.H) continue;
-      const int pi = ((r + KH / 2) * PW + c + KW / 2) * PXS + FCL::cbo(cb);
-      if (PREC) {
-        float f[8];
-        join8(patch[pi], patch[NPP + pi], patch[2 * NPP + pi], f);
-        st_chunk(xo + (long)i * 8, f);
-      } else {
-        *reinterpret_cast<uint4*>(xo + (long)i * 8) = patch[pi];
-      }
-    }
-  }
+          *reinterpret_cast<uint4*>(xo + o) = patch[pi];
+        }
+      }
+    }
+  };
+  stage(std::integral_constant<int, 0>(), std::integral_constant<int, FCL::NC0>());
   for (int c = tid; c < NKS * 4; c += NTH) {
     int kk, cb;
     ent(c, kk, cb);
-    coff[c] = c < NCH ? ((kk / KW) * PW + (kk % KW)) * PXS + FCL::cbo(cb) : 0;
+    coff[c] = c < NCH ? ((kk / KW) * PW + (kk % KW)) * PXS + FCL::cbo(FCL::cloc(cb)) : 0;
   }
 #pragma unroll
   for (int s = 0; s < PF; ++s) load_a(s, areg[s]);
@@ -353,18 +363,47 @@
     const int c = s * 4 + kq;
     int kk, cb;
     ent(c, kk, cb);
-    return c < NCH ? ((kk / KW) * PW + (kk % KW)) * PXS + FCL::cbo(cb) : 0;
-  };
-  auto load_b = [&](int s, uint4 (*dst)[NPL]) {
+    return c < NCH ? ((kk / KW) * PW + (kk % KW)) * PXS + FCL::cbo(FCL::cloc(cb)) : 0;
+  };
+  auto load_bn = [&](int s, int h0, auto n_, uint4 (*dst)[NPL]) {
     const uint4* pb = patch + lbase + gbase + (SCHED ? koff(s) : coff[s * 4 + kq]);
 #pragma unroll
-    for (int h = 0; h < PG; ++h) {
-      const int p = h * 16;
+    for (int h = 0; h < decltype(n_)::value; ++h) {
+      const int p = (h0 + h) * 16;
 #pragma unroll
       for (int q = 0; q < NPL; ++q) dst[h][q] = pb[q * NPP + ((p / W) * PW + (p % W)) * PXS];
     }
   };
-  if (!(a.dbg & 1)) {
+  auto load_b = [&](int s, uint4 (*dst)[NPL]) { load_bn(s, 0, std::integral_constant<int, PG>(), dst); };
+  constexpr int NBB = TWO ? 2 : 1, PGB = PG / NBB;
+  static_assert(PG % NBB == 0, "fragment batches split the wave's pixel groups evenly");
+  auto ksteps = [&](auto s0_, auto s1_, uint4 (&bfr)[2][PGB][NPL]) {
+    constexpr int Q0 = decltype(s0_)::value * NBB, Q1 = decltype(s1_)::value * NBB;
+    constexpr std::integral_constant<int, PGB> n;
+    load_bn(Q0 / NBB, 0, n, bfr[Q0 & 1]);
+#pragma unroll
+    for (int q = Q0; q < Q1; ++q) {
+      const int s = q / NBB, hb = (q % NBB) * PGB;
+      if (q + 1 < Q1) load_bn((q + 1) / NBB, ((q + 1) % NBB) * PGB, n, bfr[(q + 1) & 1]);
+#pragma unroll
+      for (int t = 0; t < CT; ++t)
+#pragma unroll
+        for (int h = 0; h < PGB; ++h) acc[t][hb + h] = mma(t, areg[s % PF][t], bfr[q & 1][h], acc[t][hb + h]);
+      if (q % NBB == NBB - 1 && s + PF < NKS) load_a(s + PF, areg[s % PF]);
+    }
+  };
+  if constexpr (TWO != 0) {
+    static_assert(PARTS && PREC != 0 && !SCHED && NKS <= 64 && S2Parts<KH, KW, NCBI, W, PREC>::e0 % 4 == 0,
+                  "two-pass staging: part 0 ends on a k-step boundary of the part-major order");
+    constexpr int KS0 = S2Parts<KH, KW, NCBI, W, PREC>::e0 / 4;
+    uint4 bfr[2][PGB][NPL];
+    if (!(a.dbg & 1)) ksteps(std::integral_constant<int, 0>(), std::integral_constant<int, KS0>(), bfr);
+    asm volatile("s_waitcnt lgkmcnt(0)" ::: "memory");
+    __syncthreads();
+    stage(std::integral_constant<int, FCL::NC0>(), std::integral_constant<int, FCL::NC1>());
+    __syncthreads();
+    if (!(a.dbg & 1)) ksteps(std::integral_constant<int, KS0>(), std::integral_constant<int, NKS>(), bfr);
+  } else if (!(a.dbg & 1)) {
     if constexpr (PREC != 0 && NKS > 64) {
       static_assert(PF == 2, "k-step pairs need a 2-deep weight prefetch");
       uint4 bfr[2][PG][NPL];
@@ -399,16 +438,7 @@
       }
     } else if constexpr (PREC != 0) {
       uint4 bfr[2][PG][NPL];
-      load_b(0, bfr[0]);
-#pragma unroll
-      for (int s = 0; s < NKS; ++s) {
-        if (s + 1 < NKS) load_b(s + 1, bfr[(s + 1) & 1]);
-#pragma unroll
-        for (int t = 0; t < CT; ++t)
-#pragma unroll
-          for (int h = 0; h < PG; ++h) acc[t][h] = mma(t, areg[s % PF][t], bfr[s & 1][h], acc[t][h]);
-        if (s + PF < NKS) load_a(s + PF, areg[s % PF]);
-      }
+      ksteps(std::integral_constant<int, 0>(), std::integral_constant<int, NKS>(), bfr);
     } else {
 #pragma unroll
       for (int s = 0; s < NKS; ++s) {
diff --git a/gentun_amd/models/cnn_hip.py b/gentun_amd/models/cnn_hip.py
--- a/gentun_amd/models/cnn_hip.py
+++ b/gentun_amd/models/cnn_hip.py
@@ -16,6 +16,8 @@
 WINOGRAD = False
 
 WFRAG = True
+
+TWOPASS = True
 
 EVAL_TWIN_BUDGET = 1 << 30
 
@@ -268,10 +270,11 @@
             L.part_b = torch.zeros((L.S, Q, L.coutp), dtype=torch.float32, device=dev)
         self.wino_tr = K.WinoTransform(wsegs, dev) if wsegs else None
         fspecs = []
+        frag_on = WFRAG and K.fast_path_on(self.L)
         for L in self.layers:
             first = L.slots == ["input"]
             L.wfrag = L.wfragT = False
-            if not WFRAG or L.wino:
+            if not frag_on or L.wino:
                 continue
             nr = max(1, len(L.rows))
             if K._probe_conv(self.L, L.KH, L.KW, L.cinp, L.coutp, L.H, L.W, self.prec, nr, B, L.cout, True):
@@ -379,6 +382,11 @@
         a.prec = self.prec
         a.wps = w[0].numel()
         return a
+
+    def _set_twopass(self, a):
+        a.twopass = 1 if TWOPASS and K.fast_path_on(self.L) else 0
+        if a.twopass and self.L.gt_conv_fast_twopass(a) != 1:
+            a.twopass = 0
 
     def _bn_args(self, L, train, pools=()):
         a = K.BnArgs()
@@ -424,6 +432,7 @@
             a.epi_bf16 = 1
             if cpools:
                 a.pool_y, a.pool_mask = self.act[st.pool].data_ptr(), st.pmask.data_ptr()
+            self._set_twopass(a)
             ops.append(("conv", a, L))
             if self.bn:
                 b = self._bn_args(L, 1, pools)
@@ -579,6 +588,7 @@
                         a.pool_y, a.pool_mask = self.grad[st.inp].data_ptr(), st.pmask.data_ptr()
                         a.unpool_x1 = self.grad[self.sched.pool_x1(st)].data_ptr()
                         a.unpool_sel = st.sel.data_ptr()
+                    self._set_twopass(a)
                     return a
                 a = None
                 if fuse_bwd and len(L.slots) == 1 and L.slots[0] in pool_stage:
@@ -871,6 +881,7 @@
                 b.pool_y = rp(b.pool_y or 0)
                 b.pool_mask = 0
                 b.B = EB
+                self._set_twopass(b)
                 ops.append((kind, b, Lr))
             elif kind == "bn":
                 b = K.BnArgs.from_buffer_copy(a)
diff --git a/gentun_amd/ops/cnn_kernels.py b/gentun_amd/ops/cnn_kernels.py
--- a/gentun_amd/ops/cnn_kernels.py
+++ b/gentun_amd/ops/cnn_kernels.py
@@ -25,7 +25,7 @@
                 ("G", I), ("B", I), ("H", I), ("W", I), ("Cinp", I), ("Coutp", I), ("KH", I), ("KW", I),
                 ("TH", I), ("ngroups", I), ("xsum", P), ("dbg", I), ("epi_bf16", I), ("prec", I), ("wps", C.c_long),
                 ("cbb", I), ("pool_y", P), ("pool_mask", P), ("unpool_x1", P), ("unpool_sel", P),
-                ("cout_real", I), ("Hr", I), ("Wr", I), ("wino", I), ("wfrag", I)]
+                ("cout_real", I), ("Hr", I), ("Wr", I), ("wino", I), ("wfrag", I), ("twopass", I)]
 
 
 class WinoWSeg(C.Structure):
@@ -252,6 +252,10 @@
         L.gt_conv_fast_probe_any.restype = I
         L.gt_conv_fast_select.argtypes = [C.POINTER(ConvArgs), C.POINTER(ConvSel)]
         L.gt_conv_fast_select.restype = I
+        L.gt_conv_fast_twopass.argtypes = [C.POINTER(ConvArgs)]
+        L.gt_conv_fast_twopass.restype = I
+        L.gt_conv_fast_occupancy.argtypes = [C.POINTER(ConvArgs)]
+        L.gt_conv_fast_occupancy.restype = I
         L.gt_wgrad_fast_select.argtypes = [C.POINTER(WgradArgs), C.POINTER(WgradSel)]
         L.gt_wgrad_fast_select.restype = I
         L.gt_sizeof_conv_sel.restype = C.c_size_t
```

New measurement: 1085, median of 6. +2.8%, better.
